# Andreas-Edling/raytracer-rs

Measured on AMD Instinct MI355X. Metric: Mrays/s (whole node) + ms/frame, 1920x1080x64spp thai2.dae, higher is better.
Workload: dtype f32

## Files before the change

### include/mi355rt.h

```cpp
#ifndef MI355RT_H
#define MI355RT_H

#include <stddef.h>
#include <stdint.h>

#ifdef __cplusplus
extern "C" {
#endif

#define MI355RT_OK            0
#define MI355RT_E_INVALID    -1
#define MI355RT_E_NO_DEVICE  -2
#define MI355RT_E_LOAD       -3
#define MI355RT_E_HIP        -4

#define MI355RT_DEFAULT_TRIANGLES_PER_LEAF 70u
#define MI355RT_DEFAULT_STRIPE_ROWS 4u

#define MI355RT_FLAG_FIX_ROW_INDEX  1u
#define MI355RT_FLAG_COUNT_STEPS    2u
#define MI355RT_FLAG_TIME_KERNELS   4u
#define MI355RT_FLAG_OCTREE_SEMANTICS 8u
#define MI355RT_FLAG_TRUE_CLOSEST_HIT 32u
#define MI355RT_FLAG_GROUP_SHARES_DEVICE 16u
#define MI355RT_FLAG_DEVICE_LBVH 64u
#define MI355RT_FLAG_DIRECT_FILM 128u

typedef struct mi355rt_handle mi355rt_handle;

typedef struct mi355rt_material {
    uint32_t kind;
    float rgb[3];
    uint32_t tex_id;
} mi355rt_material;

typedef struct mi355rt_light {
    float pos[3];
    float color[3];
} mi355rt_light;

typedef struct mi355rt_texture {
    uint32_t width, height;
    const float* rgb;
} mi355rt_texture;

typedef struct mi355rt_scene_desc {
    const float* tri_verts;
    const uint32_t* tri_geom;
    uint32_t ntri;
    const mi355rt_material* materials;
    uint32_t nmaterials;
    const mi355rt_light* lights;
    uint32_t nlights;
    const mi355rt_texture* textures;
    uint32_t ntextures;
    float camera_orientation[16];
    float camera_fov_deg;
} mi355rt_scene_desc;

typedef struct mi355rt_config {
    uint32_t width, height;
    uint32_t triangles_per_leaf;
    uint32_t recursions;
    uint32_t spread;
    uint32_t flags;
    uint64_t seed;
    int32_t device;
    uint32_t stripe_rows, stripe_rank, stripe_world;
    uint32_t samples_per_pass;
    uint32_t device_count;
} mi355rt_config;

typedef struct mi355rt_ray_counts {
    uint64_t primary;
    uint64_t bounce;
    uint64_t shadow;
    uint64_t primary_hits;
    uint64_t primary_culled;
    uint64_t nodes_visited;
    uint64_t tris_tested;
    uint64_t trace_launches;
    uint64_t inner_execs;
    uint64_t leaf_execs;
    double trace_ms;
    double total_ms;
    double trace_secondary_ms;
    uint64_t trace_secondary_launches;
    double shader_clock_mhz;
    uint64_t shadow_skipped;
} mi355rt_ray_counts;

void mi355rt_default_config(mi355rt_config* cfg);

int mi355rt_create(const mi355rt_scene_desc* scene, const mi355rt_config* cfg, mi355rt_handle** out);
int mi355rt_create_from_collada_str(const char* doc, size_t len, const char* data_dir,
                                    const mi355rt_config* cfg, mi355rt_handle** out);
int mi355rt_create_from_collada_file(const char* path, const mi355rt_config* cfg, mi355rt_handle** out);
int mi355rt_create_from_scene_file(const char* path, const mi355rt_config* cfg, mi355rt_handle** out);
void mi355rt_destroy(mi355rt_handle* h);

const char* mi355rt_last_error(const mi355rt_handle* h);

uint32_t mi355rt_trace_frame_additive(mi355rt_handle* h);
int mi355rt_render(mi355rt_handle* h, uint32_t spp, mi355rt_ray_counts* counts);
int mi355rt_render_async(mi355rt_handle* h, uint32_t spp);
int mi355rt_last_counts(mi355rt_handle* h, mi355rt_ray_counts* counts);

#define MI355RT_ADAPTIVE_TILE 8u
typedef struct mi355rt_adaptive_config {
    uint32_t min_spp;
    uint32_t max_spp;
    uint32_t batch_spp;
    uint32_t max_rounds;
    float rel_error;
    float abs_floor;
} mi355rt_adaptive_config;

typedef struct mi355rt_adaptive_stats {
    uint32_t rounds;
    uint32_t tiles;
    uint32_t tiles_active_first;
    uint32_t tiles_active_last;
    uint64_t samples_added;
} mi355rt_adaptive_stats;

void mi355rt_adaptive_default_config(mi355rt_adaptive_config* cfg);
int mi355rt_render_adaptive(mi355rt_handle* h, const mi355rt_adaptive_config* cfg, mi355rt_adaptive_stats* stats);
int mi355rt_adaptive_tile_mask(mi355rt_handle* h, const mi355rt_adaptive_config* cfg, uint8_t* out, size_t ntiles);

typedef struct mi355rt_denoise_config {
    uint32_t iterations;
    uint32_t normal_power_log2;
    float sigma_luminance;
    float sigma_depth;
    float sigma_albedo;
} mi355rt_denoise_config;
void mi355rt_denoise_default_config(mi355rt_denoise_config* cfg);
int mi355rt_get_denoised_pixels(mi355rt_handle* h, const mi355rt_denoise_config* cfg, float* rgb, uint32_t* packed, size_t npix);
int mi355rt_film_get_direct(mi355rt_handle* h, float* sum_rgb);
int mi355rt_get_denoised_pixels_split(mi355rt_handle* h, const mi355rt_denoise_config* cfg, float* rgb, uint32_t* packed, size_t npix);
int mi355rt_get_guides(mi355rt_handle* h, float* depth, float* normal3, float* albedo3, uint32_t* prim, size_t npix);

#define MI355RT_DISPLAY_SOURCE_FILM            0u
#define MI355RT_DISPLAY_SOURCE_DENOISED        1u
#define MI355RT_DISPLAY_SOURCE_DENOISED_SPLIT  2u
#define MI355RT_CURVE_REINHARD        0u
#define MI355RT_CURVE_REINHARD_WHITE  1u
#define MI355RT_CURVE_ACES            2u
#define MI355RT_CURVE_CLAMP           3u
#define MI355RT_TRANSFER_REFERENCE    0u
#define MI355RT_TRANSFER_SRGB         1u
#define MI355RT_HIST_BINS 256u

typedef struct mi355rt_luminance_histogram {
    uint32_t bins[MI355RT_HIST_BINS];
    uint32_t empty;
    uint32_t nan;
    uint32_t nonpositive;
    uint32_t max_bits;
} mi355rt_luminance_histogram;

typedef struct mi355rt_display_config {
    uint32_t source, curve, transfer;
    uint32_t auto_exposure;
    float exposure;
    float white;
    float key, low, high;
} mi355rt_display_config;

void mi355rt_display_default_config(mi355rt_display_config* cfg);
int mi355rt_display_histogram(mi355rt_handle* h, uint32_t source, const mi355rt_denoise_config* dn, mi355rt_luminance_histogram* out);
int mi355rt_display_auto_exposure(const mi355rt_luminance_histogram* hist, float key, float low, float high, float* exposure);
int mi355rt_display_srgb_thresholds(float out[255]);
int mi355rt_get_display_pixels(mi355rt_handle* h, const mi355rt_display_config* cfg, const mi355rt_denoise_config* dn,
                               uint32_t* packed, size_t npix, float* exposure_used );

int mi355rt_get_tonemapped_pixels(mi355rt_handle* h, uint32_t* out, size_t n);
int mi355rt_tonemap_owned_rows_device(mi355rt_handle* h, uint32_t* device_out, size_t n);
int mi355rt_tonemap_owned_rows_device_on_stream(mi355rt_handle* h, uint32_t* device_out, size_t n, void* hip_stream);
uint32_t mi355rt_owned_rows(const mi355rt_handle* h);
int mi355rt_owned_row_list(const mi355rt_handle* h, uint32_t* rows, size_t n);

int mi355rt_film_get(mi355rt_handle* h, float* sum_rgb, float* sumsq_rgb, uint32_t* n);
int mi355rt_film_clear(mi355rt_handle* h);
int mi355rt_film_get_pixels(mi355rt_handle* h, float* rgb);
int mi355rt_film_get_estimated_variances(mi355rt_handle* h, float* rgb);

int mi355rt_film_set(mi355rt_handle* h, const float* sum_rgb, const float* sumsq_rgb, const uint32_t* n, const float* direct_rgb, size_t npix);
int mi355rt_film_add(mi355rt_handle* h, const float* sum_rgb, const float* sumsq_rgb, const uint32_t* n, const float* direct_rgb, size_t npix);
int mi355rt_film_save(mi355rt_handle* h, const char* path);
int mi355rt_film_load(mi355rt_handle* h, const char* path, int add);
int mi355rt_film_file_info(const char* path, uint32_t out[8]);

int mi355rt_camera_move_rel(mi355rt_handle* h, float x, float y, float z);
int mi355rt_camera_add_x_angle(mi355rt_handle* h, float radians);
int mi355rt_camera_add_y_angle(mi355rt_handle* h, float radians);
int mi355rt_camera_get(const mi355rt_handle* h, float rot16[16], float orient16[16], float max_xy[2]);
int mi355rt_camera_get_ray(const mi355rt_handle* h, uint32_t u, uint32_t v, float xi1, float xi2, float ray6[6]);

int mi355rt_set_seed(mi355rt_handle* h, uint64_t seed);
int mi355rt_set_flags(mi355rt_handle* h, uint32_t flags);
int mi355rt_set_slices(mi355rt_handle* h, uint32_t slices);
uint32_t mi355rt_get_slices(const mi355rt_handle* h);

int mi355rt_intersect_rays(mi355rt_handle* h, const float* rays6, size_t n, float* tuv, uint32_t* prim);
int mi355rt_occluded_rays(mi355rt_handle* h, const float* rays6, size_t n, uint8_t* blocked);

#define MI355RT_RAYS_HOST   0u
#define MI355RT_RAYS_DEVICE 1u
typedef struct mi355rt_ray_outputs {
    float*    rgb;
    float*    direct;
    float*    tuv;
    uint32_t* prim;
} mi355rt_ray_outputs;
int mi355rt_trace_rays(mi355rt_handle* h, const float* rays6, const uint32_t* keys2 ,
                       size_t n, uint32_t where, const mi355rt_ray_outputs* out);
int mi355rt_render_rays(mi355rt_handle* h, const float* rays6, size_t nrays, uint32_t spp, uint32_t where, mi355rt_ray_counts* counts);

int mi355rt_get_sample_table(const mi355rt_handle* h, float* out);
int mi355rt_debug_sample(mi355rt_handle* h, uint32_t pixel, uint32_t sampleno, float color3[3], float* node_L, size_t nodes);
int mi355rt_debug_numerics(mi355rt_handle* h, const float* a, const float* b, size_t n, float* quot, float* root, float* pow32);
int mi355rt_debug_slab(mi355rt_handle* h, const float* inv_rays6, const float* cubes6, size_t n, uint8_t* hit, float* tmin);
uint32_t mi355rt_tree_nodes(const mi355rt_handle* h);
int mi355rt_debug_speculation(const mi355rt_handle* h, uint64_t out[2]);
int mi355rt_debug_light_map(const float* tri_verts, uint32_t ntri, const float light[3], double pad, uint32_t res, float* out_dist2, double* nearest);

int mi355rt_debug_wide_bvh(const float* tri_verts, uint32_t ntri, uint32_t out[8]);

int mi355rt_accel_stats(const mi355rt_handle* h, uint32_t out[8]);
int mi355rt_bvh_build_info(const mi355rt_handle* h, uint32_t out[2]);
int mi355rt_octree_stats(const mi355rt_handle* h, uint32_t out[8]);
uint32_t mi355rt_device_count(const mi355rt_handle* h);
int mi355rt_debug_gather_rate(mi355rt_handle* h, uint32_t table_nodes, uint32_t steps, double out[3]);
int64_t mi355rt_debug_check_guards(mi355rt_handle* h);
uint64_t mi355rt_hbm_allocated_bytes(const mi355rt_handle* h);
int mi355rt_synchronize(mi355rt_handle* h);

#define MI355RT_COMM_ID_BYTES 128
int mi355rt_comm_unique_id(uint8_t* id128);
int mi355rt_comm_available(mi355rt_handle* h);
int mi355rt_comm_init(mi355rt_handle* h, const uint8_t* id128);
int mi355rt_comm_gather_frame(mi355rt_handle* h, uint32_t root, uint32_t* host_out, size_t n);
int mi355rt_comm_destroy(mi355rt_handle* h);
uint32_t mi355rt_comm_ranks(mi355rt_handle* h);

uint32_t mi355rt_width(const mi355rt_handle* h);
uint32_t mi355rt_height(const mi355rt_handle* h);
uint32_t mi355rt_triangle_count(const mi355rt_handle* h);
uint32_t mi355rt_current_row(const mi355rt_handle* h);

#ifdef __cplusplus
}
#endif
#endif
```

### raytracer-rs_amd/__init__.py

```python
import ctypes as C
import os
import sys
import time
import weakref

import numpy as np

DEFAULT_TRIANGLES_PER_LEAF = 70

FLAG_FIX_ROW_INDEX = 1
FLAG_COUNT_STEPS = 2
FLAG_TIME_KERNELS = 4
FLAG_OCTREE_SEMANTICS = 8
FLAG_GROUP_SHARES_DEVICE = 16
FLAG_TRUE_CLOSEST_HIT = 32
FLAG_DEVICE_LBVH = 64
FLAG_DIRECT_FILM = 128

_HERE = os.path.dirname(os.path.abspath(__file__))
LIB_PATH = os.environ.get("MI355RT_LIB") or os.path.join(_HERE, "libmi355rt.so")
_lib = None


class Material(C.Structure):
    _fields_ = [("kind", C.c_uint32), ("rgb", C.c_float * 3), ("tex_id", C.c_uint32)]


class Light(C.Structure):
    _fields_ = [("pos", C.c_float * 3), ("color", C.c_float * 3)]


class Texture(C.Structure):
    _fields_ = [("width", C.c_uint32), ("height", C.c_uint32), ("rgb", C.POINTER(C.c_float))]


class SceneDesc(C.Structure):
    _fields_ = [
        ("tri_verts", C.POINTER(C.c_float)), ("tri_geom", C.POINTER(C.c_uint32)), ("ntri", C.c_uint32),
        ("materials", C.POINTER(Material)), ("nmaterials", C.c_uint32),
        ("lights", C.POINTER(Light)), ("nlights", C.c_uint32),
        ("textures", C.POINTER(Texture)), ("ntextures", C.c_uint32),
        ("camera_orientation", C.c_float * 16), ("camera_fov_deg", C.c_float),
    ]


class Config(C.Structure):
    _fields_ = [
        ("width", C.c_uint32), ("height", C.c_uint32), ("triangles_per_leaf", C.c_uint32),
        ("recursions", C.c_uint32), ("spread", C.c_uint32), ("flags", C.c_uint32),
        ("seed", C.c_uint64), ("device", C.c_int32),
        ("stripe_rows", C.c_uint32), ("stripe_rank", C.c_uint32), ("stripe_world", C.c_uint32),
        ("samples_per_pass", C.c_uint32), ("device_count", C.c_uint32),
    ]


class RayCounts(C.Structure):
    _fields_ = [
        ("primary", C.c_uint64), ("bounce", C.c_uint64), ("shadow", C.c_uint64), ("primary_hits", C.c_uint64),
        ("primary_culled", C.c_uint64),
        ("nodes_visited", C.c_uint64), ("tris_tested", C.c_uint64), ("trace_launches", C.c_uint64),
        ("inner_execs", C.c_uint64), ("leaf_execs", C.c_uint64),
        ("trace_ms", C.c_double), ("total_ms", C.c_double),
        ("trace_secondary_ms", C.c_double), ("trace_secondary_launches", C.c_uint64), ("shader_clock_mhz", C.c_double),
        ("shadow_skipped", C.c_uint64),
    ]

    def as_dict(self):
        d = {name: getattr(self, name) for name, _ in self._fields_}
        d["total_rays"] = self.primary + self.bounce + self.shadow
        d["traced_rays"] = d["total_rays"] - self.primary_culled - self.shadow_skipped
        return d


ADAPTIVE_TILE = 8


class AdaptiveConfig(C.Structure):
    _fields_ = [("min_spp", C.c_uint32), ("max_spp", C.c_uint32), ("batch_spp", C.c_uint32), ("max_rounds", C.c_uint32),
                ("rel_error", C.c_float), ("abs_floor", C.c_float)]


class AdaptiveStats(C.Structure):
    _fields_ = [("rounds", C.c_uint32), ("tiles", C.c_uint32), ("tiles_active_first", C.c_uint32), ("tiles_active_last", C.c_uint32),
                ("samples_added", C.c_uint64)]

    def as_dict(self):
        return {name: int(getattr(self, name)) for name, _ in self._fields_}


class DenoiseConfig(C.Structure):
    _fields_ = [("iterations", C.c_uint32), ("normal_power_log2", C.c_uint32),
                ("sigma_luminance", C.c_float), ("sigma_depth", C.c_float), ("sigma_albedo", C.c_float)]


HIST_BINS = 256
DISPLAY_SOURCE_FILM, DISPLAY_SOURCE_DENOISED, DISPLAY_SOURCE_DENOISED_SPLIT = 0, 1, 2
CURVE_REINHARD, CURVE_REINHARD_WHITE, CURVE_ACES, CURVE_CLAMP = 0, 1, 2, 3
TRANSFER_REFERENCE, TRANSFER_SRGB = 0, 1


class LuminanceHistogram(C.Structure):
    _fields_ = [("bins", C.c_uint32 * HIST_BINS), ("empty", C.c_uint32), ("nan", C.c_uint32), ("nonpositive", C.c_uint32), ("max_bits", C.c_uint32)]

    def as_dict(self):
        return dict(bins=np.array(self.bins, np.uint32), empty=int(self.empty), nan=int(self.nan), nonpositive=int(self.nonpositive), max_bits=int(self.max_bits))

    @classmethod
    def from_dict(cls, d):
        h = cls()
        bins = np.ascontiguousarray(d["bins"], np.uint32).reshape(HIST_BINS)
        C.memmove(h.bins, bins.ctypes.data, HIST_BINS * 4)
        h.empty, h.nan, h.nonpositive, h.max_bits = (int(d.get(k, 0)) for k in ("empty", "nan", "nonpositive", "max_bits"))
        return h


class DisplayConfig(C.Structure):
    _fields_ = [("source", C.c_uint32), ("curve", C.c_uint32), ("transfer", C.c_uint32), ("auto_exposure", C.c_uint32),
                ("exposure", C.c_float), ("white", C.c_float), ("key", C.c_float), ("low", C.c_float), ("high", C.c_float)]


RAYS_HOST, RAYS_DEVICE = 0, 1


class RayOutputs(C.Structure):
    _fields_ = [("rgb", C.c_void_p), ("direct", C.c_void_p), ("tuv", C.c_void_p), ("prim", C.c_void_p)]


RAY_OUTPUTS = ("rgb", "direct", "tuv", "prim")

_H = C.c_void_p
_F = C.POINTER(C.c_float)
_U = C.POINTER(C.c_uint32)
ABI = [
    ("mi355rt_default_config", None, [C.POINTER(Config)]),
    ("mi355rt_create", C.c_int, [C.POINTER(SceneDesc), C.POINTER(Config), C.POINTER(_H)]),
    ("mi355rt_create_from_collada_str", C.c_int, [C.c_char_p, C.c_size_t, C.c_char_p, C.POINTER(Config), C.POINTER(_H)]),
    ("mi355rt_create_from_collada_file", C.c_int, [C.c_char_p, C.POINTER(Config), C.POINTER(_H)]),
    ("mi355rt_create_from_scene_file", C.c_int, [C.c_char_p, C.POINTER(Config), C.POINTER(_H)]),
    ("mi355rt_destroy", None, [_H]),
    ("mi355rt_last_error", C.c_char_p, [_H]),
    ("mi355rt_trace_frame_additive", C.c_uint32, [_H]),
    ("mi355rt_render", C.c_int, [_H, C.c_uint32, C.POINTER(RayCounts)]),
    ("mi355rt_render_async", C.c_int, [_H, C.c_uint32]),
    ("mi355rt_last_counts", C.c_int, [_H, C.POINTER(RayCounts)]),
    ("mi355rt_adaptive_default_config", None, [C.POINTER(AdaptiveConfig)]),
    ("mi355rt_render_adaptive", C.c_int, [_H, C.POINTER(AdaptiveConfig), C.POINTER(AdaptiveStats)]),
    ("mi355rt_adaptive_tile_mask", C.c_int, [_H, C.POINTER(AdaptiveConfig), C.POINTER(C.c_uint8), C.c_size_t]),
    ("mi355rt_denoise_default_config", None, [C.POINTER(DenoiseConfig)]),
    ("mi355rt_get_denoised_pixels", C.c_int, [_H, C.POINTER(DenoiseConfig), _F, _U, C.c_size_t]),
    ("mi355rt_film_get_direct", C.c_int, [_H, _F]),
    ("mi355rt_get_denoised_pixels_split", C.c_int, [_H, C.POINTER(DenoiseConfig), _F, _U, C.c_size_t]),
    ("mi355rt_get_guides", C.c_int, [_H, _F, _F, _F, _U, C.c_size_t]),
    ("mi355rt_display_default_config", None, [C.POINTER(DisplayConfig)]),
    ("mi355rt_display_histogram", C.c_int, [_H, C.c_uint32, C.POINTER(DenoiseConfig), C.POINTER(LuminanceHistogram)]),
    ("mi355rt_display_auto_exposure", C.c_int, [C.POINTER(LuminanceHistogram), C.c_float, C.c_float, C.c_float, _F]),
    ("mi355rt_display_srgb_thresholds", C.c_int, [_F]),
    ("mi355rt_get_display_pixels", C.c_int, [_H, C.POINTER(DisplayConfig), C.POINTER(DenoiseConfig), _U, C.c_size_t, _F]),
    ("mi355rt_get_tonemapped_pixels", C.c_int, [_H, _U, C.c_size_t]),
    ("mi355rt_tonemap_owned_rows_device", C.c_int, [_H, C.c_void_p, C.c_size_t]),
    ("mi355rt_tonemap_owned_rows_device_on_stream", C.c_int, [_H, C.c_void_p, C.c_size_t, C.c_void_p]),
    ("mi355rt_owned_rows", C.c_uint32, [_H]),
    ("mi355rt_owned_row_list", C.c_int, [_H, _U, C.c_size_t]),
    ("mi355rt_film_get", C.c_int, [_H, _F, _F, _U]),
    ("mi355rt_film_clear", C.c_int, [_H]),
    ("mi355rt_film_set", C.c_int, [_H, _F, _F, _U, _F, C.c_size_t]),
    ("mi355rt_film_add", C.c_int, [_H, _F, _F, _U, _F, C.c_size_t]),
    ("mi355rt_film_save", C.c_int, [_H, C.c_char_p]),
    ("mi355rt_film_load", C.c_int, [_H, C.c_char_p, C.c_int]),
    ("mi355rt_film_file_info", C.c_int, [C.c_char_p, _U]),
    ("mi355rt_film_get_pixels", C.c_int, [_H, _F]),
    ("mi355rt_film_get_estimated_variances", C.c_int, [_H, _F]),
    ("mi355rt_camera_move_rel", C.c_int, [_H, C.c_float, C.c_float, C.c_float]),
    ("mi355rt_camera_add_x_angle", C.c_int, [_H, C.c_float]),
    ("mi355rt_camera_add_y_angle", C.c_int, [_H, C.c_float]),
    ("mi355rt_camera_get", C.c_int, [_H, _F, _F, _F]),
    ("mi355rt_camera_get_ray", C.c_int, [_H, C.c_uint32, C.c_uint32, C.c_float, C.c_float, _F]),
    ("mi355rt_set_seed", C.c_int, [_H, C.c_uint64]),
    ("mi355rt_set_flags", C.c_int, [_H, C.c_uint32]),
    ("mi355rt_set_slices", C.c_int, [_H, C.c_uint32]),
    ("mi355rt_get_slices", C.c_uint32, [_H]),
    ("mi355rt_intersect_rays", C.c_int, [_H, _F, C.c_size_t, _F, _U]),
    ("mi355rt_occluded_rays", C.c_int, [_H, _F, C.c_size_t, C.POINTER(C.c_uint8)]),
    ("mi355rt_trace_rays", C.c_int, [_H, C.c_void_p, C.c_void_p, C.c_size_t, C.c_uint32, C.POINTER(RayOutputs)]),
    ("mi355rt_render_rays", C.c_int, [_H, C.c_void_p, C.c_size_t, C.c_uint32, C.c_uint32, C.POINTER(RayCounts)]),
    ("mi355rt_get_sample_table", C.c_int, [_H, _F]),
    ("mi355rt_debug_sample", C.c_int, [_H, C.c_uint32, C.c_uint32, _F, _F, C.c_size_t]),
    ("mi355rt_debug_numerics", C.c_int, [_H, _F, _F, C.c_size_t, _F, _F, _F]),
    ("mi355rt_debug_slab", C.c_int, [_H, _F, _F, C.c_size_t, C.POINTER(C.c_uint8), _F]),
    ("mi355rt_tree_nodes", C.c_uint32, [_H]),
    ("mi355rt_debug_speculation", C.c_int, [_H, C.POINTER(C.c_uint64)]),
    ("mi355rt_debug_light_map", C.c_int, [_F, C.c_uint32, _F, C.c_double, C.c_uint32, _F, C.POINTER(C.c_double)]),
    ("mi355rt_debug_wide_bvh", C.c_int, [_F, C.c_uint32, _U]),
    ("mi355rt_accel_stats", C.c_int, [_H, _U]),
    ("mi355rt_octree_stats", C.c_int, [_H, _U]),
    ("mi355rt_bvh_build_info", C.c_int, [_H, _U]),
    ("mi355rt_device_count", C.c_uint32, [_H]),
    ("mi355rt_synchronize", C.c_int, [_H]),
    ("mi355rt_comm_unique_id", C.c_int, [C.POINTER(C.c_uint8)]),
    ("mi355rt_comm_available", C.c_int, [_H]),
    ("mi355rt_comm_init", C.c_int, [_H, C.POINTER(C.c_uint8)]),
    ("mi355rt_comm_gather_frame", C.c_int, [_H, C.c_uint32, _U, C.c_size_t]),
    ("mi355rt_comm_destroy", C.c_int, [_H]),
    ("mi355rt_comm_ranks", C.c_uint32, [_H]),
    ("mi355rt_hbm_allocated_bytes", C.c_uint64, [_H]),
    ("mi355rt_debug_check_guards", C.c_int64, [_H]),
    ("mi355rt_debug_gather_rate", C.c_int, [_H, C.c_uint32, C.c_uint32, C.POINTER(C.c_double)]),
    ("mi355rt_width", C.c_uint32, [_H]),
    ("mi355rt_height", C.c_uint32, [_H]),
    ("mi355rt_triangle_count", C.c_uint32, [_H]),
    ("mi355rt_current_row", C.c_uint32, [_H]),
]


def lib():
    global _lib
    if _lib is None:
        if not os.path.exists(LIB_PATH):
            raise ImportError(
                "libmi355rt.so is not built (%s); run __graft_entry__.build() — there is no CPU fallback" % LIB_PATH)
        if "torch" in sys.modules:
            try:
                sys.modules["torch"].cuda.is_available()
            except Exception:
                pass
        L = C.CDLL(LIB_PATH)
        for name, res, args in ABI:
            fn = getattr(L, name)
            fn.restype = res
            fn.argtypes = args
        _lib = L
    return _lib


def _fp(a):
    return a.ctypes.data_as(_F)


def _up(a):
    return a.ctypes.data_as(_U)


def _is_tensor(a):
    t = sys.modules.get("torch")
    return t is not None and isinstance(a, t.Tensor)


def _ray_array(a, name, cols, dtype, rows=None):
    want = np.dtype(dtype).name
    if _is_tensor(a):
        if a.device.type != "cuda":
            raise ValueError("%s: a torch tensor must live on the handle's GPU (it is on %s); pass a numpy array for host memory" % (name, a.device))
        if str(a.dtype).replace("torch.", "") not in ((want, "int32") if want == "uint32" else (want,)):
            raise TypeError("%s: dtype must be %s, not %s" % (name, want, a.dtype))
        shape, contiguous, addr, dev = tuple(a.shape), a.is_contiguous(), a.data_ptr(), True
    elif isinstance(a, np.ndarray):
        if a.dtype != np.dtype(dtype):
            raise TypeError("%s: dtype must be %s, not %s" % (name, want, a.dtype))
        shape, contiguous, addr, dev = a.shape, a.flags["C_CONTIGUOUS"], a.ctypes.data, False
    else:
        raise TypeError("%s: a numpy array or a torch tensor, not %s" % (name, type(a).__name__))
    if len(shape) != 2 or shape[1] != cols or (rows is not None and shape[0] != rows):
        raise ValueError("%s: shape must be (%s, %d), not %s" % (name, "n" if rows is None else rows, cols, tuple(shape)))
    if not contiguous:
        raise ValueError("%s: must be C-contiguous" % name)
    return addr, shape[0], dev


def default_config(width=1024, height=768, **kw):
    cfg = Config()
    lib().mi355rt_default_config(C.byref(cfg))
    cfg.width, cfg.height = int(width), int(height)
    for k, v in kw.items():
        if not hasattr(cfg, k):
            raise TypeError("unknown config field %r" % k)
# ... 287 lines not shown
        else:
            self._check(lib().mi355rt_tonemap_owned_rows_device(self._h, C.c_void_p(device_ptr), n))

    def intersect_rays(self, rays6):
        rays6 = np.ascontiguousarray(rays6, np.float32).reshape(-1, 6)
        n = rays6.shape[0]
        tuv = np.zeros((n, 3), np.float32); prim = np.zeros(n, np.uint32)
        self._check(lib().mi355rt_intersect_rays(self._h, _fp(rays6), n, _fp(tuv), _up(prim)))
        return tuv, prim

    def trace_rays(self, rays6, keys=None, want=("rgb",)):
        want = tuple(want)
        if not want or any(w not in RAY_OUTPUTS for w in want) or len(set(want)) != len(want):
            raise ValueError("want: a non-empty selection of %s without repeats, not %r" % (RAY_OUTPUTS, want))
        addr, n, dev = _ray_array(rays6, "rays6", 6, np.float32)
        kaddr = None
        if keys is not None:
            kaddr, _, kdev = _ray_array(keys, "keys", 2, np.uint32, rows=n)
            if kdev != dev:
                raise ValueError("keys must live where rays6 lives (both numpy arrays, or both tensors on the GPU)")
        res, o = {}, RayOutputs()
        if dev:
            import torch
            torch.cuda.current_stream(rays6.device).synchronize()
            for w in want:
                res[w] = torch.zeros((n,) if w == "prim" else (n, 3), dtype=torch.int32 if w == "prim" else torch.float32, device=rays6.device)
                setattr(o, w, res[w].data_ptr())
            torch.cuda.current_stream(rays6.device).synchronize()
        else:
            for w in want:
                res[w] = np.zeros(n, np.uint32) if w == "prim" else np.zeros((n, 3), np.float32)
                setattr(o, w, res[w].ctypes.data)
        self._check(lib().mi355rt_trace_rays(self._h, addr, kaddr, n, RAYS_DEVICE if dev else RAYS_HOST, C.byref(o)))
        return res

    def render_rays(self, rays6, spp):
        spp = int(spp)
        if spp < 1:
            raise ValueError("spp must be >= 1")
        addr, n, dev = _ray_array(rays6, "rays6", 6, np.float32, rows=self.width * self.height * spp)
        if dev:
            import torch
            torch.cuda.current_stream(rays6.device).synchronize()
        rc = RayCounts()
        self._check(lib().mi355rt_render_rays(self._h, addr, n, spp, RAYS_DEVICE if dev else RAYS_HOST, C.byref(rc)))
        return rc

    def occluded_rays(self, rays6):
        rays6 = np.ascontiguousarray(rays6, np.float32).reshape(-1, 6)
        n = rays6.shape[0]
        out = np.zeros(n, np.uint8)
        self._check(lib().mi355rt_occluded_rays(self._h, _fp(rays6), n, out.ctypes.data_as(C.POINTER(C.c_uint8))))
        return out

    def sample_table(self):
        out = np.zeros((65536, 3), np.float32)
        self._check(lib().mi355rt_get_sample_table(self._h, _fp(out)))
        return out

    def debug_sample(self, pixel, sampleno):
        nodes = lib().mi355rt_tree_nodes(self._h)
        color = np.zeros(3, np.float32); node_l = np.zeros((nodes, 3), np.float32)
        self._check(lib().mi355rt_debug_sample(self._h, pixel, sampleno, _fp(color), _fp(node_l), nodes))
        return color, node_l

    def debug_numerics(self, a, b):
        a = np.ascontiguousarray(a, np.float32); b = np.ascontiguousarray(b, np.float32)
        q = np.zeros_like(a); r = np.zeros_like(a); p = np.zeros_like(a)
        self._check(lib().mi355rt_debug_numerics(self._h, _fp(a), _fp(b), a.size, _fp(q), _fp(r), _fp(p)))
        return q, r, p

    def debug_slab(self, inv_rays6, cubes6):
        r = np.ascontiguousarray(inv_rays6, np.float32).reshape(-1, 6); c = np.ascontiguousarray(cubes6, np.float32).reshape(-1, 6)
        assert r.shape == c.shape
        hit = np.zeros(r.shape[0], np.uint8); tmin = np.zeros(r.shape[0], np.float32)
        self._check(lib().mi355rt_debug_slab(self._h, _fp(r), _fp(c), r.shape[0], hit.ctypes.data_as(C.POINTER(C.c_uint8)), _fp(tmin)))
        return hit.astype(bool), tmin

    def accel_stats(self):
        out = np.zeros(8, np.uint32)
        self._check(lib().mi355rt_accel_stats(self._h, _up(out)))
        return dict(nodes=int(out[0]), leaves=int(out[1]), max_depth=int(out[2]), max_leaf=int(out[3]),
                    node_bytes=int(out[4]), tri_bytes=int(out[5]), bvh_build_ms=int(out[6]) / 1000.0, octree_build_ms=int(out[7]) / 1000.0)

    def bvh_build_info(self):
        out = np.zeros(2, np.uint32)
        self._check(lib().mi355rt_bvh_build_info(self._h, _up(out)))
        return dict(on_device=bool(out[0]), device_ms=int(out[1]) / 1000.0)

    def octree_stats(self):
        out = np.zeros(8, np.uint32)
        self._check(lib().mi355rt_octree_stats(self._h, _up(out)))
        return dict(nodes=int(out[0]), inner=int(out[1]), leaves=int(out[2]), empty=int(out[3]), depth=int(out[4]), tri_refs=int(out[5]))

    @property
    def triangle_count(self):
        return lib().mi355rt_triangle_count(self._h)

    @property
    def current_row(self):
        return lib().mi355rt_current_row(self._h)


def _finish(code, handle, keep=None):
    if code != 0:
        raise RuntimeError((lib().mi355rt_last_error(None) or b"").decode() or "mi355rt error %d" % code)
    return RayTracer(handle.value, keep)


def create_raytracer(collada_doc, triangles_per_leaf, width, height, data_dir=None, **cfg_kw):
    cfg = default_config(width, height, triangles_per_leaf=triangles_per_leaf, **cfg_kw)
    doc = collada_doc.encode() if isinstance(collada_doc, str) else bytes(collada_doc)
    h = C.c_void_p()
    code = lib().mi355rt_create_from_collada_str(doc, len(doc), data_dir.encode() if data_dir else None, C.byref(cfg), C.byref(h))
    return _finish(code, h)


def create_raytracer_from_file(collada_filename, triangles_per_leaf, width, height, **cfg_kw):
    cfg = default_config(width, height, triangles_per_leaf=triangles_per_leaf, **cfg_kw)
    h = C.c_void_p()
    code = lib().mi355rt_create_from_collada_file(str(collada_filename).encode(), C.byref(cfg), C.byref(h))
    return _finish(code, h)


def create_raytracer_from_scene_file(scene_filename, triangles_per_leaf, width, height, **cfg_kw):
    cfg = default_config(width, height, triangles_per_leaf=triangles_per_leaf, **cfg_kw)
    h = C.c_void_p()
    code = lib().mi355rt_create_from_scene_file(str(scene_filename).encode(), C.byref(cfg), C.byref(h))
    return _finish(code, h)


def create_raytracer_from_arrays(scene, triangles_per_leaf, width, height, **cfg_kw):
    cfg = default_config(width, height, triangles_per_leaf=triangles_per_leaf, **cfg_kw)
    verts = np.ascontiguousarray(scene["tri_verts"], np.float32).reshape(-1)
    geom = np.ascontiguousarray(scene["tri_geom"], np.uint32)
    nm = len(scene["mat_kind"])
    mats = (Material * max(nm, 1))()
    for i in range(nm):
        mats[i].kind = int(scene["mat_kind"][i]); mats[i].tex_id = int(scene["mat_tex"][i])
        for c in range(3):
            mats[i].rgb[c] = float(scene["mat_rgb"][i][c])
    nl = len(scene["lights"])
    lights = (Light * max(nl, 1))()
    for i in range(nl):
        for c in range(3):
            lights[i].pos[c] = float(scene["lights"][i][c]); lights[i].color[c] = float(scene["lights"][i][3 + c])
    nt = len(scene["textures"])
    texs = (Texture * max(nt, 1))()
    keep = [verts, geom, mats, lights, texs]
    for i, t in enumerate(scene["textures"]):
        arr = np.ascontiguousarray(t, np.float32)
        keep.append(arr)
        texs[i].height, texs[i].width = arr.shape[0], arr.shape[1]
        texs[i].rgb = _fp(arr)
    sd = SceneDesc()
    sd.tri_verts = _fp(verts); sd.tri_geom = _up(geom); sd.ntri = geom.size
    sd.materials = mats; sd.nmaterials = nm; sd.lights = lights; sd.nlights = nl
    sd.textures = texs; sd.ntextures = nt
    for i in range(16):
        sd.camera_orientation[i] = float(scene["camera_matrix"][i])
    sd.camera_fov_deg = float(scene["camera_fov"])
    h = C.c_void_p()
    code = lib().mi355rt_create(C.byref(sd), C.byref(cfg), C.byref(h))
    return _finish(code, h, keep)


def film_file_info(path):
    out = (C.c_uint32 * 8)()
    if lib().mi355rt_film_file_info(os.fsencode(path), out) != 0:
        raise RuntimeError((lib().mi355rt_last_error(None) or b"").decode() or "mi355rt_film_file_info failed")
    return dict(version=int(out[0]), width=int(out[1]), height=int(out[2]), planes=int(out[3]), seed=int(out[4]) | int(out[5]) << 32, flags=int(out[6]))


def debug_light_map(tri_verts, light, pad, res):
    v = np.ascontiguousarray(tri_verts, np.float32).reshape(-1, 9)
    l = np.ascontiguousarray(light, np.float32).reshape(3)
    out = np.zeros((6, res, res), np.float32); nearest = C.c_double(0.0)
    code = lib().mi355rt_debug_light_map(_fp(v), v.shape[0], _fp(l), float(pad), int(res), _fp(out), C.byref(nearest))
    if code != 0:
        raise RuntimeError("mi355rt_debug_light_map failed: %d" % code)
    return out, nearest.value


def debug_wide_bvh(tri_verts):
    v = np.ascontiguousarray(tri_verts, np.float32).reshape(-1, 9)
    out = (C.c_uint32 * 8)()
    code = lib().mi355rt_debug_wide_bvh(_fp(v), v.shape[0], out)
    if code != 0:
        raise RuntimeError("mi355rt_debug_wide_bvh failed: %d" % code)
    keys = ("wide_nodes", "binary_nodes", "stack_need", "binary_depth", "children", "tris_once_wide", "bad_boxes", "tris_once_binary")
    return dict(zip(keys, (int(x) for x in out)))


def comm_unique_id():
    buf = (C.c_uint8 * 128)()
    if lib().mi355rt_comm_unique_id(buf) != 0:
        raise RuntimeError((lib().mi355rt_last_error(None) or b"").decode() or "mi355rt_comm_unique_id failed")
    return bytes(buf)


class Stats:

    def __init__(self):
        self.last_iteration = time.perf_counter()
        self.fps_sum = 0.0
        self.primrays_per_sec_sum = 0.0
        self.num_measurements = 0

    def stats(self, num_primary_rays):
        now = time.perf_counter()
        dt = now - self.last_iteration
        self.last_iteration = now
        fps = 1.0 / dt
        self.fps_sum += fps
        prs = num_primary_rays / dt
        self.primrays_per_sec_sum += prs
        self.num_measurements += 1
        return "fps: %s  primary rays/s: %d" % (fps, int(prs))

    def mean_stats(self):
        return "mean fps: %s  mean primary rays/s: %s" % (
            self.fps_sum / self.num_measurements, self.primrays_per_sec_sum / self.num_measurements)


class stats:
    Stats = Stats
```

### raytracer-rs_amd/csrc/capi.cpp

```cpp
#include <cmath>
#include <cstdio>
#include <cstring>
#include <memory>
#include <string>
#include <vector>
#include "display.hpp"
#include "lightmap.hpp"
#include "../../include/mi355rt.h"
#include "group.hpp"
#include "renderer.hpp"

using namespace mi355rt;

namespace mi355rt { bool comm_unique_id(uint8_t* id128, std::string& err); }

struct mi355rt_handle {
    std::unique_ptr<DeviceGroup> g;
    Renderer* r;
    std::string error;
};

namespace {
thread_local std::string g_create_error;

int finish_create(const SceneData& scene, const mi355rt_config* cfg, mi355rt_handle** out)
{
    int code = MI355RT_E_INVALID;
    std::string err;
    std::unique_ptr<DeviceGroup> g = DeviceGroup::create(scene, *cfg, err, code);
    if (!g) { g_create_error = err; return code; }
    Renderer* r = g->primary();
    *out = new mi355rt_handle{ std::move(g), r, std::string() };
    return MI355RT_OK;
}
int bad(const char* msg) { g_create_error = msg; return MI355RT_E_INVALID; }

bool adaptive_args_ok(mi355rt_handle* h, const mi355rt_adaptive_config* c)
{
    if (!h) return false;
    const char* e = nullptr;
    if (h->g->size() > 1) e = "adaptive sampling: not available on a device group (config.device_count > 1)";
    else if (!c) e = "adaptive sampling: null config";
    else if (c->min_spp < 2) e = "adaptive sampling: min_spp must be >= 2";
    else if (c->max_spp < c->min_spp) e = "adaptive sampling: max_spp must be >= min_spp";
    else if (c->batch_spp < 1) e = "adaptive sampling: batch_spp must be >= 1";
    else if (!std::isfinite(c->rel_error) || c->rel_error < 0.0f) e = "adaptive sampling: rel_error must be finite and >= 0";
    else if (!std::isfinite(c->abs_floor) || c->abs_floor < 0.0f) e = "adaptive sampling: abs_floor must be finite and >= 0";
    if (!e) return true;
    h->r->last_error = e;
    return false;
}

bool denoise_handle_ok(mi355rt_handle* h, size_t npix)
{
    if (!h) return false;
    const char* e = nullptr;
    if (h->g->size() > 1) e = "denoise: not available on a device group (config.device_count > 1)";
    else if (h->r->cfg.stripe_world > 1) e = "denoise: not available on a striped handle (stripe_world > 1): a stripe's neighbours belong to other ranks";
    else if (npix < (size_t)h->r->cfg.width * h->r->cfg.height) e = "denoise: output buffer too small: npix must be >= width * height";
    if (!e) return true;
    h->r->last_error = e;
    return false;
}
bool denoise_config_ok(mi355rt_handle* h, const mi355rt_denoise_config* c)
{
    const char* e = nullptr;
    auto sigma_ok = [](float s) { return std::isfinite(s) && s > 0.0f; };
    if (!c) e = "denoise: null config";
    else if (c->iterations > 10) e = "denoise: iterations must be <= 10";
    else if (c->normal_power_log2 > 10) e = "denoise: normal_power_log2 must be <= 10";
    else if (!sigma_ok(c->sigma_luminance)) e = "denoise: sigma_luminance must be finite and > 0";
    else if (!sigma_ok(c->sigma_depth)) e = "denoise: sigma_depth must be finite and > 0";
    else if (!sigma_ok(c->sigma_albedo)) e = "denoise: sigma_albedo must be finite and > 0";
    if (!e) return true;
    h->r->last_error = e;
    return false;
}
bool display_handle_ok(mi355rt_handle* h, uint32_t source)
{
    if (!h) return false;
    const char* e = nullptr;
    if (h->g->size() > 1) e = "display: not available on a device group (config.device_count > 1)";
    else if (h->r->cfg.stripe_world > 1) e = "display: not available on a striped handle (stripe_world > 1): add the stripes into one handle first";
    else if (source > MI355RT_DISPLAY_SOURCE_DENOISED_SPLIT) e = "display: unknown source";
    else if (source == MI355RT_DISPLAY_SOURCE_DENOISED_SPLIT && !h->r->has_direct_film()) e = "display: source DENOISED_SPLIT needs a handle created with MI355RT_FLAG_DIRECT_FILM";
    if (!e) return true;
    h->r->last_error = e;
    return false;
}
const char* display_key_range_error(float key, float low, float high)
// ... 478 lines not shown
    return h->g->set_seed(seed) ? MI355RT_OK : MI355RT_E_HIP;
}
int mi355rt_set_flags(mi355rt_handle* h, uint32_t flags)
{
    if (!h) return MI355RT_E_INVALID;
    return h->g->set_flags(flags) ? MI355RT_OK : MI355RT_E_INVALID;
}

int mi355rt_set_slices(mi355rt_handle* h, uint32_t slices)
{
    if (!h || slices < 1 || slices > 8) return MI355RT_E_INVALID;
    h->g->set_slices(slices);
    return MI355RT_OK;
}
uint32_t mi355rt_get_slices(const mi355rt_handle* h) { return h ? h->r->slices : 0; }

int mi355rt_intersect_rays(mi355rt_handle* h, const float* rays6, size_t n, float* tuv, uint32_t* prim)
{
    if (!h || (n && (!rays6 || !tuv || !prim))) return MI355RT_E_INVALID;
    return h->r->intersect(rays6, n, tuv, prim, nullptr) ? MI355RT_OK : MI355RT_E_HIP;
}
int mi355rt_occluded_rays(mi355rt_handle* h, const float* rays6, size_t n, uint8_t* blocked)
{
    if (!h || (n && (!rays6 || !blocked))) return MI355RT_E_INVALID;
    return h->r->intersect(rays6, n, nullptr, nullptr, blocked) ? MI355RT_OK : MI355RT_E_HIP;
}

int mi355rt_trace_rays(mi355rt_handle* h, const float* rays6, const uint32_t* keys2, size_t n, uint32_t where, const mi355rt_ray_outputs* out)
{
    if (!ray_call_ok(h, "mi355rt_trace_rays", rays6, n, where)) return MI355RT_E_INVALID;
    if (!out || (!out->rgb && !out->direct && !out->tuv && !out->prim)) { h->r->last_error = "mi355rt_trace_rays: out is NULL or every output pointer in it is NULL"; return MI355RT_E_INVALID; }
    if (n > 0xFFFFFFFFull) { h->r->last_error = "mi355rt_trace_rays: n must fit 32 bits"; return MI355RT_E_INVALID; }
    return h->r->trace_rays(rays6, keys2, n, where == MI355RT_RAYS_DEVICE, *out) ? MI355RT_OK : MI355RT_E_HIP;
}

int mi355rt_render_rays(mi355rt_handle* h, const float* rays6, size_t nrays, uint32_t spp, uint32_t where, mi355rt_ray_counts* counts)
{
    if (!ray_call_ok(h, "mi355rt_render_rays", rays6, nrays, where)) return MI355RT_E_INVALID;
    const char* e = nullptr;
    if (spp == 0) e = "mi355rt_render_rays: spp must be >= 1";
    else if (nrays != (size_t)h->r->cfg.width * h->r->cfg.height * spp) e = "mi355rt_render_rays: nrays must equal width * height * spp";
    if (e) { h->r->last_error = e; return MI355RT_E_INVALID; }
    const bool ok = h->r->render_rays(rays6, spp, where == MI355RT_RAYS_DEVICE);
    if (counts) *counts = h->r->counts;
    return ok ? MI355RT_OK : MI355RT_E_HIP;
}

int mi355rt_get_sample_table(const mi355rt_handle* h, float* out)
{
    if (!h || !out) return MI355RT_E_INVALID;
    std::memcpy(out, h->r->table.data(), h->r->table.size() * sizeof(float));
    return MI355RT_OK;
}

int mi355rt_debug_sample(mi355rt_handle* h, uint32_t pixel, uint32_t sampleno, float color3[3], float* node_L, size_t nodes)
{
    if (!h || !color3 || !node_L) return MI355RT_E_INVALID;
    return h->r->debug_sample(pixel, sampleno, color3, node_L, nodes) ? MI355RT_OK : MI355RT_E_HIP;
}
int mi355rt_debug_numerics(mi355rt_handle* h, const float* a, const float* b, size_t n, float* quot, float* root, float* pow32)
{
    if (!h || (n && (!a || !b || !quot || !root || !pow32))) return MI355RT_E_INVALID;
    return h->r->debug_numerics(a, b, n, quot, root, pow32) ? MI355RT_OK : MI355RT_E_HIP;
}
int mi355rt_debug_slab(mi355rt_handle* h, const float* inv_rays6, const float* cubes6, size_t n, uint8_t* hit, float* tmin)
{
    if (!h || (n && (!inv_rays6 || !cubes6 || !hit || !tmin))) return MI355RT_E_INVALID;
    return h->r->debug_slab(inv_rays6, cubes6, n, hit, tmin) ? MI355RT_OK : MI355RT_E_HIP;
}
uint32_t mi355rt_tree_nodes(const mi355rt_handle* h) { return h ? h->r->nodes_per_sample : 0u; }
int mi355rt_debug_speculation(const mi355rt_handle* h, uint64_t out[2])
{
    if (!h || !out) return MI355RT_E_INVALID;
    h->r->speculation_stats(out);
    return MI355RT_OK;
}
int mi355rt_debug_light_map(const float* tri_verts, uint32_t ntri, const float light[3], double pad, uint32_t res, float* out_dist2, double* nearest)
{
    if ((ntri && !tri_verts) || !light || !out_dist2 || res == 0 || res > 4096 || !(pad >= 0.0)) return MI355RT_E_INVALID;
    mi355rt::LightMap lm;
    mi355rt::build_light_map(tri_verts, ntri, light, pad, res, lm);
    std::memcpy(out_dist2, lm.dist2.data(), lm.dist2.size() * sizeof(float));
    if (nearest) *nearest = lm.nearest;
    return MI355RT_OK;
}

namespace {
struct WideWalk {
    const mi355rt::Bvh& b; std::vector<uint32_t> seen; uint32_t children = 0, bad_boxes = 0;
    void below(int32_t ref, double mn[3], double mx[3])
    {
        for (int a = 0; a < 3; ++a) { mn[a] = 1e300; mx[a] = -1e300; }
        if (ref < 0) {
            const uint32_t code = ~(uint32_t)ref, first = code >> 3, cnt = (code & 7u) + 1u;
            for (uint32_t t = first; t < first + cnt && t < b.tris.size(); ++t) {
                const mi355rt::BvhTri& r = b.tris[t];
                if (r.prim < seen.size()) ++seen[r.prim];
                for (int v = 0; v < 3; ++v) for (int a = 0; a < 3; ++a) {
                    const double x = (double)r.v0[a] + (v == 1 ? (double)r.e1[a] : v == 2 ? (double)r.e2[a] : 0.0);
                    mn[a] = std::min(mn[a], x); mx[a] = std::max(mx[a], x);
                }
            }
            return;
        }
        const mi355rt::BvhNode4& o = b.nodes4[(size_t)ref];
        const uint32_t cbm = (o.bases & 0xFFFFFu) - 128u, nb = ~(((o.bases >> 20) | ((o.ew >> 24) << 12)) << 3);
        const uint32_t lo[3] = { o.lox, o.loy, o.loz }, hi[3] = { o.hix, o.hiy, o.hiz };
        for (int i = 0; i < 4; ++i) {
            if (((lo[0] >> (8 * i)) & 0xFFu) > ((hi[0] >> (8 * i)) & 0xFFu)) continue;
            ++children;
            const uint32_t t = (o.meta >> (8 * i)) & 0xFFu;
            const int32_t cref = (t & 0x80u) ? (int32_t)(cbm + t) : (int32_t)(nb - t);
            double cmn[3], cmx[3];
            below(cref, cmn, cmx);
            for (int a = 0; a < 3; ++a) {
                const double scale = std::ldexp(1.0, (int)((o.ew >> (8 * a)) & 0xFFu) - 127);
                const double blo = (double)o.org[a] + (double)((lo[a] >> (8 * i)) & 0xFFu) * scale, bhi = (double)o.org[a] + (double)((hi[a] >> (8 * i)) & 0xFFu) * scale;
                if (cmn[a] <= cmx[a] && (blo > cmn[a] || bhi < cmx[a])) { ++bad_boxes; break; }
                mn[a] = std::min(mn[a], cmn[a]); mx[a] = std::max(mx[a], cmx[a]);
            }
        }
    }
};
}

int mi355rt_debug_wide_bvh(const float* tri_verts, uint32_t ntri, uint32_t out[8])
{
    if ((ntri && !tri_verts) || !out) return MI355RT_E_INVALID;
    std::vector<uint32_t> geom(std::max(ntri, 1u), 0u);
    mi355rt::Bvh b;
    mi355rt::build_bvh(tri_verts, geom.data(), ntri, b);
    mi355rt::build_wide(b);
    for (int k = 0; k < 8; ++k) out[k] = 0u;
    out[1] = (uint32_t)b.nodes.size(); out[3] = b.max_depth;
    if (b.nodes4.empty()) return MI355RT_OK;
    out[0] = (uint32_t)b.nodes4.size(); out[2] = b.stack_need4;
    WideWalk w{ b, std::vector<uint32_t>(ntri, 0u) };
    double mn[3], mx[3];
    w.below(0, mn, mx);
    out[4] = w.children; out[6] = w.bad_boxes;
    for (uint32_t c : w.seen) out[5] += c == 1u ? 1u : 0u;
    std::vector<uint32_t> seen2(ntri, 0u);
    std::vector<int32_t> st(1, b.root);
    while (!st.empty()) {
        const int32_t r = st.back(); st.pop_back();
        if (r < 0) { const uint32_t code = ~(uint32_t)r, first = code >> 3, cnt = (code & 7u) + 1u; for (uint32_t t = first; t < first + cnt && t < b.tris.size(); ++t) if (b.tris[t].prim < ntri) ++seen2[b.tris[t].prim]; }
        else { st.push_back(b.nodes[(size_t)r].child0); st.push_back(b.nodes[(size_t)r].child1); }
    }
    for (uint32_t c : seen2) out[7] += c == 1u ? 1u : 0u;
    return MI355RT_OK;
}

int mi355rt_accel_stats(const mi355rt_handle* h, uint32_t out[8])
{
    if (!h || !out) return MI355RT_E_INVALID;
    const Bvh& b = h->r->bvh;
    out[0] = (uint32_t)b.nodes.size(); out[1] = b.leaves; out[2] = b.max_depth; out[3] = b.max_leaf;
    out[4] = (uint32_t)(b.nodes.size() * sizeof(BvhNode)); out[5] = (uint32_t)(b.tris.size() * sizeof(BvhTri));
    out[6] = (uint32_t)(h->r->build_ms_[0] * 1000.0); out[7] = (uint32_t)(h->r->build_ms_[1] * 1000.0);
    return MI355RT_OK;
}
int mi355rt_bvh_build_info(const mi355rt_handle* h, uint32_t out[2])
{
    if (!h || !out) return MI355RT_E_INVALID;
    out[0] = h->r->bvh_on_device_ ? 1u : 0u; out[1] = (uint32_t)(h->r->lbvh_device_ms_ * 1000.0);
    return MI355RT_OK;
}
int mi355rt_octree_stats(const mi355rt_handle* h, uint32_t out[8])
{
    if (!h || !out) return MI355RT_E_INVALID;
    std::memcpy(out, h->r->oct_stats_, sizeof h->r->oct_stats_);
    return MI355RT_OK;
}
uint32_t mi355rt_device_count(const mi355rt_handle* h) { return h ? (uint32_t)h->g->size() : 0u; }

int mi355rt_debug_gather_rate(mi355rt_handle* h, uint32_t table_nodes, uint32_t steps, double out[3])
{
    if (!h || !out) return MI355RT_E_INVALID;
    return h->r->debug_gather_rate(table_nodes, steps, out) ? MI355RT_OK : MI355RT_E_HIP;
}

int64_t mi355rt_debug_check_guards(mi355rt_handle* h)
{
    if (!h) return -1;
    int64_t bad = 0;
    for (size_t i = 0; i < h->g->size(); ++i) { const long b = h->g->device(i)->check_guards(); if (b < 0) return -1; bad += b; }
    return bad;
}

uint64_t mi355rt_hbm_allocated_bytes(const mi355rt_handle* h)
{
    if (!h) return 0;
    uint64_t b = 0;
    for (size_t i = 0; i < h->g->size(); ++i) b += h->g->device(i)->hbm_allocated_bytes();
    return b;
}

int mi355rt_synchronize(mi355rt_handle* h)
{
    if (!h) return MI355RT_E_INVALID;
    return h->g->synchronize() ? MI355RT_OK : MI355RT_E_HIP;
}

int mi355rt_comm_unique_id(uint8_t* id128)
{
    if (!id128) return bad("null argument");
    std::string err;
    if (!comm_unique_id(id128, err)) { g_create_error = err; return MI355RT_E_HIP; }
    return MI355RT_OK;
}
int mi355rt_comm_available(mi355rt_handle* h)
{
    if (!h) return MI355RT_E_INVALID;
    if (h->g->size() > 1) { h->r->last_error = "a device group gathers inside the process; RCCL communicators are for one-device handles"; return MI355RT_E_INVALID; }
    return h->r->comm_available() ? MI355RT_OK : MI355RT_E_HIP;
}
int mi355rt_comm_init(mi355rt_handle* h, const uint8_t* id128)
{
    if (!h || !id128) return MI355RT_E_INVALID;
    if (h->g->size() > 1) { h->r->last_error = "a device group gathers inside the process; RCCL communicators are for one-device handles"; return MI355RT_E_INVALID; }
    return h->r->comm_init(id128) ? MI355RT_OK : MI355RT_E_HIP;
}
int mi355rt_comm_gather_frame(mi355rt_handle* h, uint32_t root, uint32_t* host_out, size_t n)
{
    if (!h) return MI355RT_E_INVALID;
    return h->r->comm_gather(root, host_out, n) ? MI355RT_OK : MI355RT_E_HIP;
}
int mi355rt_comm_destroy(mi355rt_handle* h)
{
    if (!h) return MI355RT_E_INVALID;
    h->r->comm_destroy();
    return MI355RT_OK;
}
uint32_t mi355rt_comm_ranks(mi355rt_handle* h) { return h ? h->r->comm_ranks() : 0u; }

uint32_t mi355rt_width(const mi355rt_handle* h) { return h ? h->r->cfg.width : 0u; }
uint32_t mi355rt_height(const mi355rt_handle* h) { return h ? h->r->cfg.height : 0u; }
uint32_t mi355rt_triangle_count(const mi355rt_handle* h) { return h ? h->r->ntri : 0u; }
uint32_t mi355rt_current_row(const mi355rt_handle* h) { return h ? h->r->current_row : 0u; }

}
```

### raytracer-rs_amd/csrc/device_types.hpp

```cpp
#pragma once
#include <cstdint>
#include <hip/hip_vector_types.h>

namespace mi355rt {

constexpr uint32_t kNumSamples = 65536;
constexpr uint32_t kSampleMax = 65535;
constexpr uint32_t kMaxRecursions = 3;
constexpr uint32_t kMaxLevels = kMaxRecursions + 1;

constexpr uint32_t kRayRecordBytes = 32;
constexpr uint32_t kShards = 64;
constexpr uint32_t kMaxRounds = kMaxRecursions + 2;
constexpr uint32_t kCullRects = 16;
constexpr uint32_t kMaxCursors = 64;
constexpr uint32_t kCtrlWordsPerRound = kMaxCursors * 16384;
constexpr uint32_t kShadeCursorOffset = 128;
constexpr uint32_t kConfirmCursorOffset = 64;
constexpr uint32_t kLiveCountOffset = 192;

struct DMaterial { float r, g, b; uint32_t kind_tex; };
struct DLight { float px, py, pz, cr, cg, cb;
                float tail2;
                float pad; };
struct DTexture { uint32_t width, height; uint64_t offset; };

struct DScene {
    const void* nodes;
    const void* tris;
    const void* normals;
    const DMaterial* materials;
    const DLight* lights;
    const DTexture* textures;
    const float* texels;
    const void* table;
    const void* oct_nodes;
    const uint32_t* oct_leaf_tris;
    const void* prim_tris;
    const int2* oct_info;
    const uint32_t* tri_home;
    const float* light_maps;
    uint32_t light_map_res;
    int32_t root;
    uint32_t nlights;
    uint32_t ntri;
    uint32_t oct_single_leaf;
    float oct_root[6];
};

struct DCamera {
    float rot[16];
    float origin[3];
    float max_x, max_y;
    uint32_t width, height;
    uint32_t cull_valid;
    float cull_rect[kCullRects][4];
    const uint32_t* cull_mask;
    float mask_x0, mask_y0, mask_inv_cx, mask_inv_cy;
    const uint2* tile_ofs;
    const uint2* tile_entries;
    uint32_t tile_cols, tile_rg, tile_nblocks;
};
constexpr uint32_t kCullGrid = 1024;

struct DPass {
    const uint32_t* rows;
    size_t qstride;
    uint2* slot_ps;
    uint32_t* hit_prim;
    uint32_t row0;
    uint32_t row_wrap;
    uint32_t npix;
    uint32_t row_group, row_group_shift;
    uint32_t nsamples;
    uint32_t spp;
    uint32_t sample_group;
    uint32_t seed;
    uint32_t flags;
    uint32_t recursions, spread;
    uint32_t nodes_per_sample;
    uint32_t nslots;
    uint32_t level_first[kMaxLevels + 1];
    uint32_t use_explicit, explicit_pixel, explicit_sampleno;
    uint32_t chunk;
    uint32_t nchunks;
    uint32_t region;
    uint32_t stack_depth;
    uint32_t list_cap;
    uint32_t tail_chunks;
    const uint32_t* block_culled;
    uint32_t cull_blocks;
    uint32_t* live;
    uint32_t* live_count;
    uint32_t live_cap;
    const uint8_t* tile_active;
    uint32_t tiles_x;
    const float* ray_in;
    const uint32_t* ray_keys;
    float4* ray_hit;
    uint32_t ray_mode, ray_base, ray_npix;
};
constexpr uint32_t kAdaptiveTile = 8;
struct AdaptiveArgs {
    uint32_t width, height, tiles_x, tiles_y;
    uint32_t stripe_rows, stripe_world, stripe_rank;
    uint32_t min_spp, max_spp, batch_spp;
    float rel_error, abs_floor;
};
constexpr uint32_t kDnHit = 1u, kDnEmpty = 2u, kDnUnknown = 4u;
struct DenoiseArgs {
    uint32_t width, height;
    uint32_t step;
    uint32_t normal_power_log2;
    float sigma_luminance, sigma_depth, sigma_albedo;
};
constexpr uint32_t kDisplayHistWords = 260u, kDisplayHistBlock = 1024u;
struct DisplayArgs {
    uint32_t curve, transfer;
    float exposure;
    float white2;
};

struct DCounters {
    unsigned long long bounce, shadow, primary_hits, nodes_visited, tris_tested;
    unsigned long long inner_execs, leaf_execs;
    unsigned int overflow;
    unsigned int pad;
    unsigned long long primary_culled;
    unsigned long long shadow_skipped;
    unsigned long long t_first_end, t_last_end, t_sum_end, t_start, n_waves;
    unsigned long long lanes_inner, lanes_leaf, lanes_done, lane_samples;
    unsigned long long t_sum_cycles, t_sum_real;
    unsigned long long visits_below[6];
    unsigned long long refills, refill_passes, refill_rays;
};

}
```

### raytracer-rs_amd/csrc/group.cpp

```cpp
#include "group.hpp"
#include <algorithm>
#include <cstring>
#include <thread>

namespace mi355rt {

std::unique_ptr<DeviceGroup> DeviceGroup::create(const SceneData& scene, const mi355rt_config& cfg_in, std::string& err, int& code)
{
    std::unique_ptr<DeviceGroup> g(new DeviceGroup());
    mi355rt_config cfg = cfg_in;
    const uint32_t n = cfg.device_count <= 1 ? 1u : cfg.device_count;
    code = MI355RT_E_INVALID;
    if (n > 64) { err = "device_count > 64"; return nullptr; }
    if (n > 1 && cfg.stripe_world > 1) { err = "a device group deals the rows itself: stripe_world must be <= 1 when device_count > 1"; return nullptr; }
    for (uint32_t i = 0; i < n; ++i) {
        mi355rt_config c = cfg;
        c.device_count = 1;
        if (n > 1) {
            c.device = (cfg.flags & MI355RT_FLAG_GROUP_SHARES_DEVICE) ? cfg.device : cfg.device + (int32_t)i;
            if (c.stripe_rows == 0) c.stripe_rows = MI355RT_DEFAULT_STRIPE_ROWS;
            c.stripe_rank = i; c.stripe_world = n;
        }
        std::unique_ptr<Renderer> r = Renderer::create(scene, c, err, code);
        if (!r) { if (n > 1) err = "device " + std::to_string(c.device) + ": " + err; return nullptr; }
        g->devs_.push_back(std::move(r));
    }
    if (n > 1) {
        for (uint32_t i = 1; i < n; ++i) {
            const int a = g->devs_[0]->cfg.device, b = g->devs_[i]->cfg.device;
            if (a == b) continue;
            int can = 0;
            if (hipDeviceCanAccessPeer(&can, b, a) == hipSuccess && can && hipSetDevice(b) == hipSuccess) {
                hipError_t e = hipDeviceEnablePeerAccess(a, 0);
                if (e != hipSuccess && e != hipErrorPeerAccessAlreadyEnabled) (void)hipGetLastError();
            }
        }
        for (uint32_t i = 0; i < n; ++i)
            if (!g->devs_[i]->gather_prepare(i == 0)) { err = g->devs_[i]->last_error; code = MI355RT_E_HIP; return nullptr; }
    }
    code = MI355RT_OK;
    return g;
}

uint32_t DeviceGroup::trace_frame_additive()
{
    error_.clear();
    uint32_t ret = 0;
    for (size_t i = 0; i < devs_.size(); ++i) {
        ret = devs_[i]->trace_frame_additive();
        if (ret == 0) { fail_from(i); return 0; }
    }
    counts_from_render_ = false;
    return ret;
}

bool DeviceGroup::render(uint32_t spp, bool wait)
{
    error_.clear();
    if (devs_.size() == 1) { counts_from_render_ = false; return primary()->render(spp, wait); }
    std::vector<char> ok(devs_.size(), 0);
    std::vector<std::thread> th;
    for (size_t i = 0; i < devs_.size(); ++i) th.emplace_back([&, i] { ok[i] = devs_[i]->render(spp) ? 1 : 0; });
    for (auto& t : th) t.join();
    counts_ = mi355rt_ray_counts{};
    for (size_t i = 0; i < devs_.size(); ++i) {
        if (!ok[i]) return fail_from(i);
        const mi355rt_ray_counts& c = devs_[i]->counts;
        counts_.primary += c.primary; counts_.bounce += c.bounce; counts_.shadow += c.shadow; counts_.shadow_skipped += c.shadow_skipped; counts_.primary_hits += c.primary_hits;
        counts_.primary_culled += c.primary_culled; counts_.nodes_visited += c.nodes_visited; counts_.tris_tested += c.tris_tested;
        counts_.trace_launches += c.trace_launches; counts_.inner_execs += c.inner_execs; counts_.leaf_execs += c.leaf_execs;
        counts_.trace_ms += c.trace_ms; counts_.total_ms = std::max(counts_.total_ms, c.total_ms);
        counts_.trace_secondary_ms += c.trace_secondary_ms; counts_.trace_secondary_launches += c.trace_secondary_launches; counts_.shader_clock_mhz = std::max(counts_.shader_clock_mhz, c.shader_clock_mhz);
    }
    counts_from_render_ = true;
    return true;
}

bool DeviceGroup::last_counts(mi355rt_ray_counts& out)
{
    error_.clear();
    if (devs_.size() == 1) return primary()->last_counts(out);
    if (counts_from_render_) { out = counts_; return true; }
    out = mi355rt_ray_counts{};
    for (size_t i = 0; i < devs_.size(); ++i) {
        mi355rt_ray_counts c{};
        if (!devs_[i]->last_counts(c)) return fail_from(i);
        out.primary += c.primary; out.bounce += c.bounce; out.shadow += c.shadow; out.shadow_skipped += c.shadow_skipped; out.primary_hits += c.primary_hits;
        out.primary_culled += c.primary_culled; out.nodes_visited += c.nodes_visited; out.tris_tested += c.tris_tested;
        out.trace_launches += c.trace_launches; out.inner_execs += c.inner_execs; out.leaf_execs += c.leaf_execs;
        out.trace_ms += c.trace_ms; out.total_ms = std::max(out.total_ms, c.total_ms);
        out.trace_secondary_ms += c.trace_secondary_ms; out.trace_secondary_launches += c.trace_secondary_launches; out.shader_clock_mhz = std::max(out.shader_clock_mhz, c.shader_clock_mhz);
    }
    return true;
}

bool DeviceGroup::get_tonemapped(uint32_t* out, size_t n)
{
    error_.clear();
    if (devs_.size() == 1) return primary()->get_tonemapped(out, n);
    Renderer* root = primary();
    for (size_t i = 1; i < devs_.size(); ++i) {
        Renderer* d = devs_[i].get();
        if (!d->tonemap_to_gather_slot()) return fail_from(i);
        const size_t bytes = d->owned_rows.size() * (size_t)d->cfg.width * 4;
        hipError_t e = bytes ? hipMemcpyPeerAsync(root->gather_slot((uint32_t)i), root->cfg.device, d->gather_slot((uint32_t)i), d->cfg.device, bytes, d->stream()) : hipSuccess;
        if (e == hipSuccess) e = hipEventRecord(d->gather_event(), d->stream());
        if (e != hipSuccess) { error_ = std::string("stripe copy to device 0: ") + hipGetErrorString(e); return false; }
    }
    if (!root->tonemap_to_gather_slot()) return fail_from(0);
    for (size_t i = 1; i < devs_.size(); ++i) {
        hipError_t e = hipStreamWaitEvent(root->stream(), devs_[i]->gather_event(), 0);
        if (e != hipSuccess) { error_ = std::string("hipStreamWaitEvent: ") + hipGetErrorString(e); return false; }
    }
    if (!root->finish_gather(out, n)) return fail_from(0);
    return true;
}

bool DeviceGroup::film_get(float* sum, float* sumsq, uint32_t* n)
{
    error_.clear();
    if (devs_.size() == 1) return primary()->film_get(sum, sumsq, n);
    const uint32_t w = primary()->cfg.width; const size_t npix = (size_t)w * primary()->cfg.height;
    std::vector<float> ts(sum ? npix * 3 : 0), tq(sumsq ? npix * 3 : 0); std::vector<uint32_t> tn(n ? npix : 0);
    for (size_t i = 0; i < devs_.size(); ++i) {
        if (!devs_[i]->film_get(sum ? ts.data() : nullptr, sumsq ? tq.data() : nullptr, n ? tn.data() : nullptr)) return fail_from(i);
        for (uint32_t r : devs_[i]->owned_rows) {
            if (sum) std::memcpy(sum + (size_t)r * w * 3, ts.data() + (size_t)r * w * 3, (size_t)w * 12);
            if (sumsq) std::memcpy(sumsq + (size_t)r * w * 3, tq.data() + (size_t)r * w * 3, (size_t)w * 12);
            if (n) std::memcpy(n + (size_t)r * w, tn.data() + (size_t)r * w, (size_t)w * 4);
        }
    }
    return true;
}

bool DeviceGroup::film_get_direct(float* sum)
{
    error_.clear();
    if (devs_.size() == 1) return primary()->film_get_direct(sum);
    const uint32_t w = primary()->cfg.width; const size_t npix = (size_t)w * primary()->cfg.height;
    std::vector<float> t(npix * 3);
    for (size_t i = 0; i < devs_.size(); ++i) {
        if (!devs_[i]->film_get_direct(t.data())) return fail_from(i);
        for (uint32_t r : devs_[i]->owned_rows) std::memcpy(sum + (size_t)r * w * 3, t.data() + (size_t)r * w * 3, (size_t)w * 12);
    }
    return true;
}

bool DeviceGroup::film_stat(bool variances, float* rgb)
{
    error_.clear();
    if (devs_.size() == 1) return primary()->film_stat(variances, rgb);
    const uint32_t w = primary()->cfg.width; const size_t npix = (size_t)w * primary()->cfg.height;
    std::vector<float> t(npix * 3);
    for (size_t i = 0; i < devs_.size(); ++i) {
        if (!devs_[i]->film_stat(variances, t.data())) return fail_from(i);
        for (uint32_t r : devs_[i]->owned_rows) std::memcpy(rgb + (size_t)r * w * 3, t.data() + (size_t)r * w * 3, (size_t)w * 12);
    }
    return true;
}

bool DeviceGroup::film_clear()
{
    error_.clear();
    for (size_t i = 0; i < devs_.size(); ++i) if (!devs_[i]->film_clear()) return fail_from(i);
    return true;
}
bool DeviceGroup::film_put(const Renderer::FilmPlanes& in, bool add)
{
    error_.clear();
    for (size_t i = 0; i < devs_.size(); ++i) if (!devs_[i]->film_put(in, add)) return fail_from(i);
// ... 27 lines not shown
```

### raytracer-rs_amd/csrc/kernels.hip

```cpp
#include <hip/hip_runtime.h>
#include <algorithm>
#include <stdint.h>
#include <stdlib.h>
#include <map>
#include <mutex>
#include <utility>
#include "device_math.hpp"
#include "device_types.hpp"
#include "kernels.hpp"
#include "traverse.hpp"

namespace mi355rt {

typedef const uint32_t __attribute__((address_space(4))) * const_u1_ptr;
constexpr int kBlock = 256;
constexpr int kWavesPerBlock = kBlock / 64;
constexpr uint32_t kMiss = 0xFFFFFFFFu;
constexpr int kPrimaryBlocks = 7;
#ifndef MI355RT_WIDE_BLOCKS
#define MI355RT_WIDE_BLOCKS 5
#endif
constexpr int kConfirmBlocks = 5;
constexpr int kShadePBlocks = 5;
constexpr int kShadePWBlocks = 4;
constexpr int kShadeSWBlocks = 5;
constexpr int kShadeSBlocks = 7;
constexpr int kInnerStepsPerIteration = 2;
constexpr uint32_t kLeafThreshold = 16;
constexpr uint32_t kRefillThreshold = 24;
constexpr uint32_t kRefillPrimary = 48;

__device__ __forceinline__ uint32_t global_wave_id() { return blockIdx.x * kWavesPerBlock + (threadIdx.x >> 6); }

constexpr uint32_t kCursorStride = kCtrlWordsPerRound / kMaxCursors;
constexpr uint32_t kMaxTries = 8u;
static_assert(kCursorStride == 16384 && kShadeCursorOffset == 2 * kConfirmCursorOffset && kLiveCountOffset == 3 * kConfirmCursorOffset, "cursor layout (device_types.hpp) and the reset loop of resolve_kernel");
struct PullState { bool first = true; uint32_t shard = 0u, tries = 0u, part = 0xFFFFFFFFu; };
struct LiveLists { const uint32_t* list = nullptr; const uint32_t* count = nullptr; uint32_t cap = 0u; };
__device__ __forceinline__ LiveLists live_lists(const DPass& ps) { LiveLists l; l.list = ps.live; l.count = ps.live_count; l.cap = ps.live_cap; return l; }
constexpr uint32_t kWholeChunk = 0xFFFFFFFFu;

constexpr uint32_t kTailSplitShift = 2;
__device__ __forceinline__ bool pull_chunk(uint32_t* cursor, uint32_t nchunks, PullState& st, uint32_t& chunk, uint32_t tail = 0u, const LiveLists live = LiveLists())
{
    if (live.list != nullptr) {
        if (st.first) { st.first = false; st.shard = global_wave_id() % kMaxCursors; }
        while (st.tries < kMaxTries) {
            const uint32_t len = ((const_u1_ptr)(uintptr_t)live.count)[(size_t)st.shard * kCursorStride + kLiveCountOffset];
            uint32_t v = 0xFFFFFFFFu;
            if (len != 0u) { if (lane_id() == 0) v = atomicAdd(&cursor[(size_t)st.shard * kCursorStride], 1u); v = bcast_first(v); }
            uint32_t j = v; st.part = kWholeChunk;
            if (tail != 0u && v != 0xFFFFFFFFu) {
                const uint32_t head = len - (tail < len ? tail : len);
                if (v >= head) { const uint32_t jj = v - head; j = head + (jj >> kTailSplitShift); st.part = jj & ((1u << kTailSplitShift) - 1u); }
            }
            if (j < len) { chunk = ((const_u1_ptr)(uintptr_t)live.list)[(size_t)st.shard * live.cap + j]; return true; }
            st.shard = (st.shard + 1u) % kMaxCursors;
            ++st.tries;
        }
        return false;
    }
    if (st.first) { st.first = false; st.shard = global_wave_id() % kMaxCursors; }
    while (st.tries < kMaxTries) {
        uint32_t v = 0u;
        if (lane_id() == 0) v = atomicAdd(&cursor[(size_t)st.shard * kCursorStride], 1u);
        v = bcast_first(v);
        if (tail != 0u) {
            const uint32_t len = st.shard < nchunks ? (nchunks - st.shard + kMaxCursors - 1u) / kMaxCursors : 0u;
            const uint32_t head = len - (tail < len ? tail : len);
            uint32_t j = v; st.part = kWholeChunk;
            if (v >= head) { const uint32_t jj = v - head; j = head + (jj >> kTailSplitShift); st.part = jj & ((1u << kTailSplitShift) - 1u); }
            if (j < len) { chunk = st.shard + j * kMaxCursors; return true; }
        } else {
            const uint32_t c = st.shard + v * kMaxCursors;
            if (c < nchunks) { chunk = c; return true; }
        }
        st.shard = (st.shard + 1u) % kMaxCursors;
        ++st.tries;
    }
    return false;
}

constexpr uint32_t kNT = 4;
typedef float v4f_t __attribute__((ext_vector_type(4)));
template <uint32_t BIT> __device__ __forceinline__ float4 ld4(const float4* p)
{
    if constexpr ((kNT >> BIT) & 1u) { const v4f_t v = __builtin_nontemporal_load((const v4f_t*)p); return make_float4(v.x, v.y, v.z, v.w); }
    else return *p;
}
template <uint32_t BIT> __device__ __forceinline__ void st4(float4* p, float4 a)
{
    if constexpr ((kNT >> BIT) & 1u) { v4f_t v; v.x = a.x; v.y = a.y; v.z = a.z; v.w = a.w; __builtin_nontemporal_store(v, (v4f_t*)p); }
// ... 505 lines not shown

template <bool PRIMARY>
__global__ __launch_bounds__(kBlock, kConfirmBlocks) void confirm_kernel(DScene sc, DCamera cam, DPass ps, const float4* __restrict__ in_q, const uint2* __restrict__ in_counts,
                                                         float4* __restrict__ hits, uint32_t* cursor, float* __restrict__ slot_L, const uint32_t* __restrict__ film_n, uint32_t shadow_only)
{
    __shared__ uint32_t s_list[kWavesPerBlock][2][128];
    const int lane = lane_id();
    uint32_t* list_r = s_list[threadIdx.x >> 6][0];
    uint32_t* list_s = s_list[threadIdx.x >> 6][1];
    uint32_t cnt = 0u;
    PullState pull; uint32_t chunk = 0u;
    while (pull_chunk(cursor, ps.nchunks, pull, chunk, 0u, PRIMARY ? LiveLists() : live_lists(ps))) {
        uint32_t n_rad = 0u, n_sh = 0u;
        if (PRIMARY) {
            n_rad = min(ps.chunk, ps.nsamples - chunk * ps.chunk);
            if (chunk_culled(cam, ps, chunk, n_rad)) continue;
        } else { const uint2 n = in_counts[chunk]; n_rad = n.x; n_sh = n.y; }
        const uint32_t n_tot = n_rad + n_sh;
        for (uint32_t it = shadow_only ? n_rad : 0u; it < n_tot; it += 64u) {
            const uint32_t i = it + (uint32_t)lane;
            const bool valid = i < n_tot;
            const uint32_t r = valid ? (uint32_t)record_index(ps, chunk, i, n_rad) : 0u;
            const bool hit = valid && ld1<3>(&ps.hit_prim[r]) != kMiss;
                uint32_t n_new;
            const uint32_t pos = wave_append(hit, cnt, n_new);
            if (hit) { list_r[pos] = r | (i >= n_rad ? 0x80000000u : 0u); if (PRIMARY) list_s[pos] = chunk * ps.chunk + i; }
            __builtin_amdgcn_wave_barrier();
            if (cnt >= 64u) {
                cnt -= 64u;
                const uint32_t code = list_r[cnt + (uint32_t)lane];
                const uint32_t si = PRIMARY ? list_s[cnt + (uint32_t)lane] : 0u;
                __builtin_amdgcn_wave_barrier();
                confirm_record<PRIMARY>(sc, cam, ps, code & 0x7FFFFFFFu, si, (code >> 31) != 0u, in_q, hits, slot_L, film_n);
            }
        }
    }
    if ((uint32_t)lane < cnt) {
        const uint32_t code = list_r[lane];
        confirm_record<PRIMARY>(sc, cam, ps, code & 0x7FFFFFFFu, PRIMARY ? list_s[lane] : 0u, (code >> 31) != 0u, in_q, hits, slot_L, film_n);
    }
}

__device__ __forceinline__ void hemisphere_walk(const float4* __restrict__ table, const f3 n, uint32_t& jx, float4& tv)
{
    for (uint32_t guard = 0u; tv.x * n.x + tv.y * n.y + tv.z * n.z <= 0.0f && guard < kNumSamples; guard += 4u) {
        const uint32_t j1 = jx + 1u == kSampleMax ? 0u : jx + 1u;
        const uint32_t j2 = j1 + 1u == kSampleMax ? 0u : j1 + 1u;
        const uint32_t j3 = j2 + 1u == kSampleMax ? 0u : j2 + 1u;
        const uint32_t j4 = j3 + 1u == kSampleMax ? 0u : j3 + 1u;
        const float4 t1 = table[j1], t2 = table[j2], t3 = table[j3], t4 = table[j4];
        const bool r1 = t1.x * n.x + t1.y * n.y + t1.z * n.z <= 0.0f, r2 = t2.x * n.x + t2.y * n.y + t2.z * n.z <= 0.0f;
        const bool r3 = t3.x * n.x + t3.y * n.y + t3.z * n.z <= 0.0f;
        const uint32_t left = kNumSamples - guard;
        if (!r1 || left == 1u) { tv = t1; jx = j1; break; }
        if (!r2 || left == 2u) { tv = t2; jx = j2; break; }
        if (!r3 || left == 3u) { tv = t3; jx = j3; break; }
        tv = t4; jx = j4;
    }
}

constexpr uint32_t kSortBins = 8;
__device__ __forceinline__ uint32_t dir_bin(const f3 d) { return (d.x < 0.0f ? 1u : 0u) | (d.y < 0.0f ? 2u : 0u) | (d.z < 0.0f ? 4u : 0u); }

__device__ __forceinline__ bool light_proves_unoccluded(const DScene& sc, uint32_t li, const DLight& lt, const f3 l)
{
    const uint32_t R = sc.light_map_res;
    if (R == 0u) return false;
    const float l2 = l.x * l.x + l.y * l.y + l.z * l.z;
    const float vx = -l.x, vy = -l.y, vz = -l.z;
    const float ax = fabsf(vx), ay = fabsf(vy), az = fabsf(vz);
    uint32_t m; float vm, va, vb;
    if (ax >= ay && ax >= az) { m = 0u; vm = vx; va = vy; vb = vz; }
    else if (ay >= az) { m = 1u; vm = vy; va = vx; vb = vz; }
    else { m = 2u; vm = vz; va = vx; vb = vy; }
    const float am = fabsf(vm);
    if (!(am > 0.0f) || !(l2 < 3.0e38f)) return false;
    const float fR = (float)R, u = div_rn(va, am), v = div_rn(vb, am);
    const int i = min(max((int)((u * 0.5f + 0.5f) * fR), 0), (int)R - 1), j = min(max((int)((v * 0.5f + 0.5f) * fR), 0), (int)R - 1);
    const uint32_t face = 2u * m + (vm < 0.0f ? 1u : 0u);
    const float bound = sc.light_maps[((size_t)(li * 6u + face) * R + (uint32_t)i) * R + (uint32_t)j];
    return (l2 * 0.98011f < bound) & (l2 * 1.0002e-4f < lt.tail2);
}

template <bool PRIMARY, class List, bool WALK = false, bool RASTER = false, bool RAYS = false>
__device__ __forceinline__ void shade_chunk(const DScene& sc, const DCamera& cam, const DPass& ps, uint32_t level, uint32_t chunk, const List list,
                                            const float4* __restrict__ in_q, uint32_t in_nrad, uint32_t& out_nrad, uint32_t& out_nshadow,
                                            const float4* __restrict__ hits,
                                            float4* __restrict__ out_q, uint2* __restrict__ out_counts,
                                            float* __restrict__ slot_L, uint32_t* __restrict__ sample_slot,
                                            const uint32_t* __restrict__ film_n, DCounters* counters,
                                            unsigned long long& acc_bounce, unsigned long long& acc_shadow, unsigned long long& acc_hits,
                                            float4* lds_hits = nullptr, unsigned long long* acc_tris = nullptr)
{
    const int lane = lane_id();
    {
        uint32_t n_rad = PRIMARY ? min(ps.chunk, ps.nsamples - chunk * ps.chunk) : in_nrad;
        const size_t base = (size_t)chunk * ps.region;
        if (PRIMARY && !RAYS && chunk_culled(cam, ps, chunk, n_rad)) {
            if (ps.block_culled == nullptr) for (uint32_t i = (uint32_t)lane; i < n_rad; i += 64u) sample_slot[chunk * ps.chunk + i] = kMiss;
            acc_hits += (unsigned long long)chunk_active_samples(cam, ps, chunk, n_rad) << 32;
            n_rad = 0u;
        }
        uint32_t cnt = 0u;
        for (uint32_t it = 0; it < n_rad; it += 64u) {
            const uint32_t i = it + (uint32_t)lane;
            bool valid;
            float4 found = make_float4(0, 0, 0, 0);
            if (RASTER) {
                f3 ro, rd; float bt, bu, bv; uint32_t bprim;
                bool in = i < n_rad;
                if (ps.tile_active != nullptr && in) { uint32_t s, p; sample_of(ps, chunk * ps.chunk + i, s, p); in = pixel_active(ps, cam.width, pass_pixel(ps, cam.width, p)); }
                const uint32_t tested = raster_tile(sc, cam, ps, film_n, chunk, it, in, ro, rd, bt, bu, bv, bprim);
                if (acc_tris) *acc_tris += (unsigned long long)tested * (unsigned long long)__popcll(__ballot(in));
                valid = in && bprim != kMiss;
                found = make_float4(bt, bu, bv, __uint_as_float(bprim));
            } else valid = i < n_rad && ld1<2>(&ps.hit_prim[base + i]) != kMiss;
            uint32_t n_new;
            const uint32_t pos = wave_append(valid, cnt, n_new);
            if (valid) list[pos] = i;
            if (RASTER && valid) lds_hits[pos] = found;
            if (PRIMARY && i < n_rad) st1<2>(&sample_slot[chunk * ps.chunk + i], valid ? chunk * ps.chunk + pos : kMiss);
            if constexpr (RAYS) { if (ps.ray_hit != nullptr && i < n_rad && !valid) ps.ray_hit[chunk * ps.chunk + i] = make_float4(0.0f, 0.0f, 0.0f, __uint_as_float(kMiss)); }
        }
        if (PRIMARY) {
            const uint32_t planes = ps.nodes_per_sample * sc.nlights, total = cnt * 3u;
            for (uint32_t q = sc.nlights; q < planes; ++q) {
                float* z = slot_L + 3ull * ((size_t)q * ps.nslots + (size_t)chunk * ps.chunk);
                float4* z4 = (float4*)z;
                for (uint32_t k = (uint32_t)lane; k < total / 4u; k += 64u) st4<2>(&z4[k], make_float4(0.0f, 0.0f, 0.0f, 0.0f));
                for (uint32_t k = (total & ~3u) + (uint32_t)lane; k < total; k += 64u) z[k] = 0.0f;
            }
        }
        __builtin_amdgcn_wave_barrier();
        uint32_t out_front = 0u, out_back = 0u, dropped = 0u, skipped = 0u;
        for (uint32_t j = 0; j < cnt; j += 64u) {
            bool active = j + (uint32_t)lane < cnt;
            const bool in_batch = active;
            f3 o = mk3(0, 0, 0), d = mk3(0, 0, 1), hp = mk3(0, 0, 0), n = mk3(0, 0, 1);
            uint32_t slot = 0u, node = 0u, pixel = 0u, sampleno = 0u, geom = 0u;
            float4 h = make_float4(0, 0, 0, 0);
            if (active) {
                const uint32_t i = list[j + (uint32_t)lane];
                h = RASTER ? lds_hits[j + (uint32_t)lane] : ld4<2>(&hits[base + i]);
                if (PRIMARY) {
                    slot = chunk * ps.chunk + j + (uint32_t)lane;
                    primary_sample<RAYS>(cam, ps, film_n, chunk * ps.chunk + i, pixel, sampleno, o, d);
                } else {
                    const float4 r0 = ld4<2>(&in_q[base + i]), r1 = ld4<2>(&in_q[ps.qstride + base + i]);
                    o = mk3(r0.x, r0.y, r0.z); d = mk3(r0.w, r1.x, r1.y);
                    slot = __float_as_uint(r1.z); node = (__float_as_uint(r1.w) >> 8) & 0xFFFFu;
                    const uint2 px = ps.slot_ps[slot];
                    pixel = px.x; sampleno = px.y;
                }
                if (PRIMARY && level < ps.recursions) ps.slot_ps[slot] = make_uint2(pixel, sampleno);
                if (WALK) {
                    float wt = h.x, wu = h.y, wv = h.z; uint32_t wprim = __float_as_uint(h.w);
                    confirm_walk(sc, o, d, wt, wu, wv, wprim);
                    h = make_float4(wt, wu, wv, __uint_as_float(wprim));
                    active = wprim != kMiss;
                }
                if constexpr (RAYS) { if (ps.ray_hit != nullptr) ps.ray_hit[chunk * ps.chunk + i] = active ? h : make_float4(0.0f, 0.0f, 0.0f, __uint_as_float(kMiss)); }
            }
            if (WALK) dropped += (uint32_t)__popcll(__ballot(j + (uint32_t)lane < cnt && !active));
            if (active) {
                hp = add3(o, sscale(h.x, d));
                const float4 nn = ((const float4*)sc.normals)[__float_as_uint(h.w)];
                n = mk3(nn.x, nn.y, nn.z);
                geom = __float_as_uint(nn.w);
            }
            for (uint32_t li = 0; li < sc.nlights; ++li) {
                bool want = false, is_free = false;
                f3 c = mk3(0, 0, 0);
                if (active) {
                    const DLight lt = sc.lights[li];
                    const f3 l = sub3(mk3(lt.px, lt.py, lt.pz), hp);
                    const f3 ln = normalized3(l);
                    const float ndl = dot3(n, ln);
                    if (!(ndl < 0.0f)) {
                        want = true;
                        is_free = light_proves_unoccluded(sc, li, lt, l);
                        const DMaterial m = sc.materials[geom];
                        f3 diffuse = mk3(m.r, m.g, m.b);
                        if (m.kind_tex & 0x80000000u) diffuse = fetch_texel(sc, m.kind_tex & 0x7FFFFFFFu, h.y, h.z);
                        const f3 view = normalized3(d);
                        const f3 refl = sub3(sscale(2.0f * ndl, n), ln);
                        const float spec = pow32(dot3(view, refl));
                        c = mk3((diffuse.x * ndl + spec) * lt.cr, (diffuse.y * ndl + spec) * lt.cg, (diffuse.z * ndl + spec) * lt.cb);
                    }
                }
                uint32_t n_new;
                const bool ray = want && !is_free;
                skipped += (uint32_t)__popcll(__ballot(want && is_free));
                const uint32_t oi = wave_append(ray, out_back, n_new);
                if (want && (!ray || out_front + oi < ps.region)) {
                    const uint32_t term = 3u * ((node * sc.nlights + li) * ps.nslots + slot);
                    if (ray) st4<2>(&out_q[base + (ps.region - 1u - oi)], make_float4(hp.x, hp.y, hp.z, __uint_as_float(term)));
                    float* dst = slot_L + term;
                    dst[0] = c.x; dst[1] = c.y; dst[2] = c.z;
                } else if (PRIMARY && in_batch) {
                    float* dst = slot_L + 3ull * ((size_t)li * ps.nslots + (size_t)chunk * ps.chunk + j + (uint32_t)lane);
                    dst[0] = 0.0f; dst[1] = 0.0f; dst[2] = 0.0f;
                }
            }
            if (level < ps.recursions) {
                const uint32_t k = ps.spread * (ps.recursions - level);
                const uint32_t index_in_level = node - ps.level_first[level];
                for (uint32_t ci = 0; ci < k; ci += 2u) {
                    const bool two = ci + 1u < k;
                    const uint32_t child0 = ps.level_first[level + 1] + index_in_level * k + ci, child1 = child0 + 1u;
                    f3 bo0 = mk3(0, 0, 0), bd0 = mk3(0, 0, 1), bo1 = bo0, bd1 = bd0;
                    if (active) {
                        const float4* __restrict__ table = (const float4*)sc.table;
                        uint32_t a0 = pixel, a1 = sampleno, a2 = 1u + child0, a3 = ps.seed;
                        pcg4d(a0, a1, a2, a3);
                        uint32_t jx0 = __umulhi(a0, 65535u), jx1 = jx0;
                        if (two) {
                            uint32_t b0 = pixel, b1 = sampleno, b2 = 1u + child1, b3 = ps.seed;
                            pcg4d(b0, b1, b2, b3);
                            jx1 = __umulhi(b0, 65535u);
                        }
                        float4 tv0 = table[jx0], tv1 = table[jx1];
                        hemisphere_walk(table, n, jx0, tv0);
                        if (two) hemisphere_walk(table, n, jx1, tv1);
                        bd0 = mk3(tv0.x, tv0.y, tv0.z); bo0 = add3(hp, sscale(0.00001f, bd0));
                        bd1 = mk3(tv1.x, tv1.y, tv1.z); bo1 = add3(hp, sscale(0.00001f, bd1));
                    }
                    uint32_t pos[2] = { 0u, 0u };
                    const uint32_t key0 = active ? dir_bin(bd0) : kSortBins, key1 = (active && two) ? dir_bin(bd1) : kSortBins;
                    for (uint32_t b = 0; b < kSortBins; ++b) {
                        const unsigned long long m0 = __ballot(key0 == b), m1 = __ballot(key1 == b);
                        if (key0 == b) pos[0] = out_front + (uint32_t)__popcll(m0 & lanemask_lt());
                        out_front += (uint32_t)__popcll(m0);
                        if (key1 == b) pos[1] = out_front + (uint32_t)__popcll(m1 & lanemask_lt());
                        out_front += (uint32_t)__popcll(m1);
                    }
                    for (uint32_t w = 0; w < (two ? 2u : 1u); ++w) {
                        const f3 bo = w ? bo1 : bo0, bd = w ? bd1 : bd0;
                        const uint32_t child_node = w ? child1 : child0;
                        const uint32_t oi = pos[w];
                        if (active && oi + out_back < ps.region + 0u) {
                            const size_t r = base + oi;
                            st4<2>(&out_q[r], make_float4(bo.x, bo.y, bo.z, bd.x));
                            st4<2>(&out_q[ps.qstride + r], make_float4(bd.y, bd.z, __uint_as_float(slot), __uint_as_float(((level + 1u) << 4) | (child_node << 8))));
                        }
                    }
                }
            }
        }
        __builtin_amdgcn_wave_barrier();
        if (out_front + out_back > ps.region) { if (lane == 0) counters->overflow = 1u; out_front = 0u; out_back = 0u; }
        if (out_counts != nullptr && lane == 0) out_counts[chunk] = make_uint2(out_front, out_back);
        out_nrad = out_front; out_nshadow = out_back;
        acc_bounce += out_front; acc_shadow += out_back + ((unsigned long long)skipped << 32); acc_hits += cnt - dropped;
    }
}

__device__ __forceinline__ void flush_shade_counters(DCounters* counters, uint32_t wave, unsigned long long acc_bounce, unsigned long long acc_shadow, unsigned long long acc_hits)
{
    if (lane_id() == 0) {
        DCounters* cs = &counters[wave % kShards];
        if (acc_bounce) atomicAdd(&cs->bounce, acc_bounce);
        if (acc_shadow & 0xFFFFFFFFull) atomicAdd(&cs->shadow, acc_shadow & 0xFFFFFFFFull);
        if (acc_shadow >> 32) atomicAdd(&cs->shadow_skipped, acc_shadow >> 32);
        if (acc_hits & 0xFFFFFFFFull) atomicAdd(&cs->primary_hits, acc_hits & 0xFFFFFFFFull);
        if (acc_hits >> 32) atomicAdd(&cs->primary_culled, acc_hits >> 32);
    }
}

template <bool PRIMARY, bool WALK, bool RASTER = false, bool RAYS = false>
__global__ __launch_bounds__(kBlock, PRIMARY ? (WALK ? kShadePWBlocks : kShadePBlocks) : (WALK ? kShadeSWBlocks : kShadeSBlocks)) void shade_kernel(DScene sc, DCamera cam, DPass ps, uint32_t level,
                                                      const float4* __restrict__ in_q, const uint2* __restrict__ in_counts,
                                                      const float4* __restrict__ hits,
                                                      float4* __restrict__ out_q, uint2* __restrict__ out_counts, uint32_t* cursor,
                                                      float* __restrict__ slot_L, uint32_t* __restrict__ sample_slot,
                                                      const uint32_t* __restrict__ film_n, DCounters* counters)
{
    extern __shared__ uint32_t s_list[];
    const LinearList list{ &s_list[(threadIdx.x >> 6) * ps.list_cap] };
    float4* lds_hits = RASTER ? (float4*)&s_list[kWavesPerBlock * ps.list_cap] + (threadIdx.x >> 6) * ps.chunk : nullptr;
    const uint32_t wave = blockIdx.x * kWavesPerBlock + (threadIdx.x >> 6);
    unsigned long long acc_bounce = 0, acc_shadow = 0, acc_hits = 0, acc_tris = 0;
    PullState pull; uint32_t chunk = 0u;
    while (pull_chunk(cursor, ps.nchunks, pull, chunk, 0u, PRIMARY ? LiveLists() : live_lists(ps))) {
        uint32_t o_rad, o_sh;
        shade_chunk<PRIMARY, LinearList, WALK, RASTER, RAYS>(sc, cam, ps, level, chunk, list, in_q, PRIMARY ? 0u : in_counts[chunk].x, o_rad, o_sh, hits, out_q, out_counts, slot_L, sample_slot, film_n, counters, acc_bounce, acc_shadow, acc_hits,
                                                       lds_hits, (RASTER && (ps.flags & 2u)) ? &acc_tris : nullptr);
        if (PRIMARY && ps.live != nullptr && (o_rad | o_sh) != 0u && lane_id() == 0) {
            const uint32_t k = chunk % kMaxCursors;
            const uint32_t at = atomicAdd(&ps.live_count[(size_t)k * kCursorStride + kLiveCountOffset], 1u);
            ps.live[(size_t)k * ps.live_cap + at] = chunk;
        }
    }
    flush_shade_counters(counters, wave, acc_bounce, acc_shadow, PRIMARY ? acc_hits : 0ull);
    if (RASTER && acc_tris && lane_id() == 0) atomicAdd(&counters[wave % kShards].tris_tested, acc_tris);
}

template <int REC>
__device__ f3 node_radiance(const float* __restrict__ L, const DPass& ps, uint32_t nlights, uint32_t level, uint32_t index)
{
    const uint32_t node = ps.level_first[level] + index;
    f3 rad = mk3(0.0f, 0.0f, 0.0f);
    for (uint32_t li = 0; li < nlights; ++li) {
        const float* p = L + 3ull * ((size_t)node * nlights + li) * ps.nslots;
        rad = add3(rad, mk3(p[0], p[1], p[2]));
    }
    if constexpr (REC == 0) {
        return rad;
    } else {
        const uint32_t k = ps.spread * (uint32_t)REC;
        f3 sum = mk3(0.0f, 0.0f, 0.0f);
        for (uint32_t c = 0; c < k; ++c) sum = add3(sum, node_radiance<REC - 1>(L, ps, nlights, level + 1, index * k + c));
        const f3 sub = vscale(sum, div_rn(1.0f, (float)k));
        return add3(rad, sub);
    }
}

template <uint32_t kResolveLanes, bool DIRECT>
__global__ __launch_bounds__(256) void resolve_kernel(DPass ps, uint32_t width, uint32_t nlights, const float* __restrict__ slot_L,
                                                     const uint32_t* __restrict__ sample_slot,
                                                     float* film_sum, float* film_sumsq, uint32_t* film_n, float* debug_color, uint32_t* ctrl, float* film_direct)
{
    if (ctrl != nullptr && blockIdx.x == 0)
        for (uint32_t i = threadIdx.x; i < kMaxRounds * kMaxCursors * 4u; i += blockDim.x)
            ctrl[(size_t)(i / (kMaxCursors * 4u)) * kCtrlWordsPerRound + (size_t)((i / 4u) % kMaxCursors) * kCursorStride + (i % 4u) * kConfirmCursorOffset] = 0u;
    const uint32_t gid = blockIdx.x * blockDim.x + threadIdx.x;
    const uint32_t j = gid % kResolveLanes;
    const bool live = gid / kResolveLanes < ps.npix;
    const uint32_t p = live ? gid / kResolveLanes : ps.npix - 1u;
    const uint32_t spp = ps.nsamples / ps.npix;
    const uint32_t pixel = ps.use_explicit ? ps.explicit_pixel : pass_pixel(ps, width, p);
    f3 sum = mk3(0, 0, 0), sumsq = mk3(0, 0, 0), direct = mk3(0, 0, 0);
    uint32_t n = 0;
    if (!ps.use_explicit) {
        sum = mk3(film_sum[3ull * pixel], film_sum[3ull * pixel + 1], film_sum[3ull * pixel + 2]);
        sumsq = mk3(film_sumsq[3ull * pixel], film_sumsq[3ull * pixel + 1], film_sumsq[3ull * pixel + 2]);
        n = film_n[pixel];
        if constexpr (DIRECT) direct = mk3(film_direct[3ull * pixel], film_direct[3ull * pixel + 1], film_direct[3ull * pixel + 2]);
    }
    const int group_lane0 = lane_id() & ~(int)(kResolveLanes - 1u);
    const bool dead = ps.block_culled != nullptr && ps.block_culled[(uint32_t)(sample_index(ps, 0u, p) / ps.chunk) % ps.cull_blocks] != 0u;
    const bool on = ps.use_explicit || pixel_active(ps, width, pixel);
    for (uint32_t s0 = 0; s0 < spp; s0 += kResolveLanes) {
        const uint32_t sl = (s0 + j < spp && !dead && on) ? sample_slot[sample_index(ps, s0 + j, p)] : 0xFFFFFFFFu;
        const float* L = slot_L + 3ull * (size_t)sl;
// ... 929 lines not shown
```

### raytracer-rs_amd/csrc/renderer.cpp

```cpp
#include "renderer.hpp"
#include "display.hpp"
#include "lightmap.hpp"
#include <algorithm>
#include <array>
#include <chrono>
#include <cmath>
#include <cstdio>
#include <cstdlib>
#include <cstring>
#include "kernels.hpp"
#include "octree.hpp"

namespace mi355rt {

namespace {
void pcg4d(uint32_t v[4])
{
    for (int i = 0; i < 4; ++i) v[i] = v[i] * 1664525u + 1013904223u;
    v[0] += v[1] * v[3]; v[1] += v[2] * v[0]; v[2] += v[0] * v[1]; v[3] += v[1] * v[2];
    for (int i = 0; i < 4; ++i) v[i] ^= v[i] >> 16;
    v[0] += v[1] * v[3]; v[1] += v[2] * v[0]; v[2] += v[0] * v[1]; v[3] += v[1] * v[2];
}
float u01(uint32_t bits) { return (float)(bits >> 9) * (1.0f / 8388608.0f); }
}

bool Renderer::fail(hipError_t e, const char* what)
{
    last_error = std::string(what) + ": " + hipGetErrorString(e);
    return false;
}
#define HIP_TRY(expr) do { hipError_t e__ = (expr); if (e__ != hipSuccess) return fail(e__, #expr); } while (0)

bool Renderer::bind()
{
    HIP_TRY(hipSetDevice(cfg.device));
    return true;
}

template <class T> bool Renderer::upload(DeviceBuffer<T>& buf, const void* src, size_t bytes)
{
    HIP_TRY(buf.alloc(bytes ? bytes : 16, &hbm_bytes_));
    if (bytes && src) HIP_TRY(hipMemcpy(buf.get(), src, bytes, hipMemcpyHostToDevice));
    else if (bytes) HIP_TRY(hipMemset(buf.get(), 0, bytes));
    return true;
}

template <class T> bool Renderer::upload(T*& dptr, const void* src, size_t bytes)
{
    scene_bufs_.emplace_back();
    if (!upload(scene_bufs_.back(), src, bytes)) return false;
    dptr = static_cast<T*>(scene_bufs_.back().get());
    return true;
}

std::unique_ptr<Renderer> Renderer::create(const SceneData& scene, const mi355rt_config& cfg, std::string& err, int& code)
{
    std::unique_ptr<Renderer> r(new Renderer());
    r->cfg = cfg;
    if (!r->init(scene, err, code)) return nullptr;
    return r;
}

void Renderer::build_sample_table(std::vector<float>& table4)
{
    table.resize((size_t)kNumSamples * 3);
    table4.assign((size_t)kNumSamples * 4, 0.0f);
    for (uint32_t i = 0; i < kNumSamples; ++i) {
        for (uint32_t attempt = 0;; ++attempt) {
            uint32_t h[4] = { i, attempt, 0xFFFFFFFFu, (uint32_t)cfg.seed };
            pcg4d(h);
            Vec3 d(u01(h[0]) * 2.0f + -1.0f, u01(h[1]) * 2.0f + -1.0f, u01(h[2]) * 2.0f + -1.0f);
            if (dot(d, d) < 1.0f) {
                Vec3 nrm = d.normalized();
                table[3 * (size_t)i] = nrm.x; table[3 * (size_t)i + 1] = nrm.y; table[3 * (size_t)i + 2] = nrm.z;
                table4[4 * (size_t)i] = nrm.x; table4[4 * (size_t)i + 1] = nrm.y; table4[4 * (size_t)i + 2] = nrm.z;
                break;
            }
        }
    }
}

bool Renderer::set_seed(uint64_t seed)
{
    if (!bind()) return false;
    if (!settle_speculation()) return false;
// ... 56 lines not shown

    ntri = scene.ntri();
    nlights_ = (uint32_t)scene.lights.size();
    camera = Camera::from_orientation_matrix(cfg.width, cfg.height, Matrix::from_array(scene.cameras[0].orientation), scene.cameras[0].fov_deg);

    const auto t_bvh = std::chrono::steady_clock::now();
    bool on_device = false;
    if (cfg.flags & MI355RT_FLAG_DEVICE_LBVH) {
        std::string why; double ms[2];
        on_device = build_bvh_device(scene.tri_verts.data(), scene.tri_geom.data(), ntri, bvh, why, ms);
        if (on_device) { lbvh_device_ms_ = ms[0]; }
        else last_error = "device LBVH not used (" + why + "): host SAH build instead";
    }
    if (!on_device) build_bvh(scene.tri_verts.data(), scene.tri_geom.data(), ntri, bvh);
    bvh_on_device_ = on_device;
    wide_ = false;
    if (kernels_walk_wide_nodes()) {
        build_wide(bvh);
        if (!bvh.nodes4.empty()) wide_ = true;
        else if (bvh.root >= 0) { err = "this build's kernels walk the 4-wide tree, which does not serve this scene"; code = MI355RT_E_INVALID; return false; }
    }
    build_ms_[0] = std::chrono::duration<double, std::milli>(std::chrono::steady_clock::now() - t_bvh).count();
    collect_cull_boxes();
    if (bvh.max_depth > kBvhMaxDepth) { err = "internal: BVH deeper than the traversal stack"; code = MI355RT_E_INVALID; return false; }
    std::vector<float> normals((size_t)std::max(ntri, 1u) * 4, 0.0f);
    for (uint32_t t = 0; t < ntri; ++t) {
        const float* v = &scene.tri_verts[9 * (size_t)t];
        Vec3 v0(v[0], v[1], v[2]), v1(v[3], v[4], v[5]), v2(v[6], v[7], v[8]);
        Vec3 n = cross(v1 - v0, v2 - v0).normalized();
        normals[4 * (size_t)t] = n.x; normals[4 * (size_t)t + 1] = n.y; normals[4 * (size_t)t + 2] = n.z;
        uint32_t g = scene.tri_geom[t];
        std::memcpy(&normals[4 * (size_t)t + 3], &g, 4);
    }
    std::vector<float> table4;
    build_sample_table(table4);
    void* d_nodes = nullptr; void* d_tris = nullptr; void* d_normals = nullptr; void* d_table = nullptr;
    DMaterial* d_mats = nullptr; DLight* d_lights = nullptr; DTexture* d_tex = nullptr; float* d_texels = nullptr;
    if (wide_ ? !upload(d_nodes, bvh.nodes4.data(), bvh.nodes4.size() * sizeof(BvhNode4)) : !upload(d_nodes, bvh.nodes.data(), bvh.nodes.size() * sizeof(BvhNode))) return bail();
    if (!upload(d_tris, bvh.tris.data(), bvh.tris.size() * sizeof(BvhTri))) return bail();
    if (!upload(d_normals, normals.data(), normals.size() * sizeof(float))) return bail();
    if (!upload(d_table, table4.data(), table4.size() * sizeof(float))) return bail();
    std::vector<DMaterial> mats(std::max<size_t>(scene.materials.size(), 1));
    for (size_t i = 0; i < scene.materials.size(); ++i) {
        const MaterialData& m = scene.materials[i];
        mats[i] = DMaterial{ m.rgb[0], m.rgb[1], m.rgb[2], m.kind == 1 ? (0x80000000u | m.tex_id) : 0u };
    }
    if (!upload(d_mats, mats.data(), mats.size() * sizeof(DMaterial))) return bail();
    std::vector<DLight> lights(std::max<size_t>(scene.lights.size(), 1));
    for (size_t i = 0; i < scene.lights.size(); ++i) {
        const LightData& l = scene.lights[i];
        lights[i] = DLight{ l.pos[0], l.pos[1], l.pos[2], l.color[0], l.color[1], l.color[2], 0.0f, 0.0f };
    }
    float* d_light_maps = nullptr; uint32_t light_map_res = 0;
    if (!scene.lights.empty() && scene.lights.size() <= 8 && ntri > 0 && !getenv("MI355RT_NO_LIGHT_MAP")) {
        const auto t_lm = std::chrono::steady_clock::now();
        double diag2 = 0.0;
        { float mn[3] = { 3e38f, 3e38f, 3e38f }, mx[3] = { -3e38f, -3e38f, -3e38f };
          for (size_t i = 0; i < scene.tri_verts.size(); ++i) { const int a = (int)(i % 3); mn[a] = std::min(mn[a], scene.tri_verts[i]); mx[a] = std::max(mx[a], scene.tri_verts[i]); }
          for (int a = 0; a < 3; ++a) diag2 += ((double)mx[a] - mn[a]) * ((double)mx[a] - mn[a]); }
        const double pad = 2e-4 * std::sqrt(diag2) + 1e-7;
        uint32_t res = 512;
        while (res > 16 && (size_t)6 * res * res * 4 * scene.lights.size() > ((size_t)64 << 20)) res /= 2;
        const uint64_t work_cap = 4ull << 20;
        for (const LightData& l : scene.lights) while (res > 16 && light_map_work(scene.tri_verts.data(), ntri, l.pos, res) > work_cap) res /= 2;
        std::vector<float> all; all.reserve((size_t)6 * res * res * scene.lights.size());
        bool finite = true;
        for (size_t i = 0; i < scene.lights.size() && finite; ++i) {
            const LightData& l = scene.lights[i];
            if (!std::isfinite(l.pos[0]) || !std::isfinite(l.pos[1]) || !std::isfinite(l.pos[2])) { finite = false; break; }
            LightMap lm; build_light_map(scene.tri_verts.data(), ntri, l.pos, pad, res, lm);
            all.insert(all.end(), lm.dist2.begin(), lm.dist2.end());
            const double tail = std::max(lm.nearest - pad, 0.0);
            lights[i].tail2 = std::isfinite(tail) ? (float)std::min(tail * tail * (1.0 - 1e-6), 3.0e38) : 3.0e38f;
            if ((double)lights[i].tail2 > tail * tail) lights[i].tail2 = std::nextafterf(lights[i].tail2, 0.0f);
        }
        if (finite) {
            if (!upload(d_light_maps, all.data(), all.size() * sizeof(float))) return bail();
            light_map_res = res;
        }
        light_map_ms_ = std::chrono::duration<double, std::milli>(std::chrono::steady_clock::now() - t_lm).count();
        if (getenv("MI355RT_DEBUG_CULL")) fprintf(stderr, "[mi355rt] light maps: %zu lights, %u texels per face edge, %.1f ms\n", scene.lights.size(), light_map_res, light_map_ms_);
    }
    if (!upload(d_lights, lights.data(), lights.size() * sizeof(DLight))) return bail();
    std::vector<DTexture> tex(std::max<size_t>(scene.textures.size(), 1));
    std::vector<float> texels;
    for (size_t i = 0; i < scene.textures.size(); ++i) {
        const TextureData& t = scene.textures[i];
        if (t.rgb.size() != (size_t)t.width * t.height * 3 || t.rgb.empty()) { err = "texture size mismatch"; code = MI355RT_E_INVALID; return false; }
        tex[i] = DTexture{ t.width, t.height, texels.size() / 3 };
        texels.insert(texels.end(), t.rgb.begin(), t.rgb.end());
    }
    if (!upload(d_tex, tex.data(), tex.size() * sizeof(DTexture))) return bail();
    if (!upload(d_texels, texels.data(), texels.size() * sizeof(float))) return bail();
    dscene_.nodes = d_nodes; dscene_.tris = d_tris; dscene_.normals = d_normals; dscene_.materials = d_mats;
    dscene_.lights = d_lights; dscene_.textures = d_tex; dscene_.texels = d_texels; dscene_.table = d_table;
    dscene_.root = bvh.root; dscene_.nlights = nlights_; dscene_.ntri = ntri;
    dscene_.light_maps = d_light_maps; dscene_.light_map_res = light_map_res;
    dscene_.oct_nodes = nullptr; dscene_.oct_leaf_tris = nullptr; dscene_.prim_tris = nullptr; dscene_.oct_info = nullptr; dscene_.tri_home = nullptr; dscene_.oct_single_leaf = 0u;
    std::memset(dscene_.oct_root, 0, sizeof dscene_.oct_root);
    mode_ = (cfg.flags & MI355RT_FLAG_OCTREE_SEMANTICS) ? kModeOctreeWalk : (cfg.flags & MI355RT_FLAG_TRUE_CLOSEST_HIT) ? kModeTrueClosest : kModeConfirm;
    if (mode_ != kModeTrueClosest) {
        Octree oct;
        const auto t_oct = std::chrono::steady_clock::now();
        build_octree(scene.tri_verts.data(), ntri, cfg.triangles_per_leaf, oct);
        build_ms_[1] = std::chrono::duration<double, std::milli>(std::chrono::steady_clock::now() - t_oct).count();
        oct_stats_[0] = (uint32_t)oct.nodes.size(); oct_stats_[1] = oct.inner; oct_stats_[2] = oct.leaves;
        oct_stats_[3] = oct.empty_leaves; oct_stats_[4] = oct.max_depth; oct_stats_[5] = (uint32_t)oct.leaf_tris.size();
        std::vector<BvhTri> prim_tris(std::max(ntri, 1u));
        std::memset(prim_tris.data(), 0, prim_tris.size() * sizeof(BvhTri));
        for (uint32_t t = 0; t < ntri; ++t) {
            const float* v = &scene.tri_verts[9 * (size_t)t];
            for (int a = 0; a < 3; ++a) { prim_tris[t].v0[a] = v[a]; prim_tris[t].e1[a] = v[3 + a] - v[a]; prim_tris[t].e2[a] = v[6 + a] - v[a]; }
            prim_tris[t].prim = t; prim_tris[t].geom = scene.tri_geom[t];
        }
        void* d_oct = nullptr; uint32_t* d_leaf = nullptr; void* d_ptris = nullptr;
        if (!upload(d_oct, oct.nodes.data(), oct.nodes.size() * sizeof(OctNodeFlat))) return bail();
        if (!upload(d_leaf, oct.leaf_tris.data(), oct.leaf_tris.size() * 4)) return bail();
        if (!upload(d_ptris, prim_tris.data(), prim_tris.size() * sizeof(BvhTri))) return bail();
        dscene_.oct_nodes = d_oct; dscene_.oct_leaf_tris = d_leaf; dscene_.prim_tris = d_ptris;
        std::vector<int2> info(oct.nodes.size());
        std::vector<uint32_t> home(std::max(ntri, 1u), 0xFFFFFFFEu);
        for (size_t i = 0; i < oct.nodes.size(); ++i) {
            const OctNodeFlat& f = oct.nodes[i];
            if (f.first_child >= 0) { info[i].x = f.first_child; info[i].y = 0; continue; }
            info[i].x = ~(int32_t)f.tri_first; info[i].y = (int32_t)f.tri_count;
            for (uint32_t k = 0; k < f.tri_count; ++k) {
                uint32_t& h = home[oct.leaf_tris[f.tri_first + k]];
                h = h == 0xFFFFFFFEu ? (uint32_t)i : 0xFFFFFFFFu;
            }
        }
        int2* d_info = nullptr; uint32_t* d_home = nullptr;
        if (!upload(d_info, info.data(), info.size() * sizeof(int2))) return bail();
        if (!upload(d_home, home.data(), home.size() * 4)) return bail();
        dscene_.oct_info = d_info; dscene_.tri_home = d_home;
        dscene_.oct_single_leaf = (mode_ == kModeConfirm && oct.nodes.size() == 1) ? 1u : 0u;
        for (int a = 0; a < 3; ++a) { dscene_.oct_root[a] = oct.nodes[0].cmin[a]; dscene_.oct_root[3 + a] = oct.nodes[0].cmax[a]; }
    }

    const size_t npix = (size_t)cfg.width * cfg.height;
    if (!upload(d_film_sum_, nullptr, npix * 12) || !upload(d_film_sumsq_, nullptr, npix * 12) || !upload(d_film_n_, nullptr, npix * 4)) return bail();
    if ((cfg.flags & MI355RT_FLAG_DIRECT_FILM) && !upload(d_film_direct_, nullptr, npix * 12)) return bail();
    if (!upload(d_ldr_, nullptr, npix * 4)) return bail();
    ldr_dirty_.assign(cfg.height, (uint8_t)1);
    if (hipEventCreateWithFlags(&ev_tonemap_, hipEventDisableTiming) != hipSuccess || hipEventCreateWithFlags(&ev_gather_, hipEventDisableTiming) != hipSuccess) { err = "hipEventCreate failed"; return false; }
    if (hipEventCreateWithFlags(&ev_call_done_, hipEventDisableTiming) != hipSuccess || hipEventCreateWithFlags(&ev_spec_done_, hipEventDisableTiming) != hipSuccess
        || hipStreamCreateWithFlags(&read_stream_, hipStreamNonBlocking) != hipSuccess) { err = "hipEventCreate / hipStreamCreate failed"; return false; }
    std::vector<uint32_t> all(cfg.height);
    for (uint32_t r = 0; r < cfg.height; ++r) {
        all[r] = r;
        if ((r / cfg.stripe_rows) % cfg.stripe_world == cfg.stripe_rank) owned_rows.push_back(r);
    }
    if (!upload(d_all_rows_, all.data(), all.size() * 4)) return bail();
    if (!upload(d_owned_rows_, owned_rows.data(), owned_rows.size() * 4)) return bail();
    if (!upload(d_tmp_rows_, nullptr, 64 * 4)) return bail();
    if (!upload(d_counters_, nullptr, sizeof(DCounters) * kShards)) return bail();
    if (h_counters_.alloc(sizeof(DCounters) * kShards) != hipSuccess) { err = "pinned host allocation failed"; return false; }
    std::memset(h_counters_.get(), 0, sizeof(DCounters) * kShards);
    slices_[0].stream = stream_;
    for (uint32_t i = 0; i < kMaxSlices; ++i) {
        if (i && hipStreamCreateWithFlags(&slices_[i].stream, hipStreamNonBlocking) != hipSuccess) { err = "hipStreamCreate failed"; return false; }
        if (hipEventCreateWithFlags(&slices_[i].done, hipEventDisableTiming) != hipSuccess) { err = "hipEventCreate failed"; return false; }
        if (!upload(slices_[i].d_ctrl, nullptr, kMaxRounds * kCtrlWordsPerRound * 4)) return bail();
        if (!upload(slices_[i].d_rows, nullptr, (size_t)cfg.height * 4)) return bail();
    }
    if (const char* e = getenv("MI355RT_SLICES")) { int v = atoi(e); if (v >= 1 && v <= (int)kMaxSlices) slices = (uint32_t)v; }
    if (!upload(d_debug_color_, nullptr, 16)) return bail();

    records_per_sample_ = 1;
    for (uint32_t l = 0; l <= cfg.recursions; ++l) {
        uint32_t nl = level_first[l + 1] - level_first[l];
        uint32_t nn = l < cfg.recursions ? level_first[l + 2] - level_first[l + 1] : 0;
        records_per_sample_ = std::max(records_per_sample_, nl * std::max(nlights_, 1u) + nn);
    }
    max_level_nodes_ = 1;
    for (uint32_t l = 0; l <= cfg.recursions; ++l) max_level_nodes_ = std::max(max_level_nodes_, level_first[l + 1] - level_first[l]);
    code = MI355RT_OK;
    return true;
}

Renderer::~Renderer()
// ... 386 lines not shown
    const bool confirm_here = mode_ == kModeConfirm && !dscene_.oct_single_leaf;
    for (uint32_t r = 0; r < cfg.recursions + 2; ++r) {
        const bool fuse_primary = r == 0 && cam.tile_ofs != nullptr && mode_ != kModeOctreeWalk;
        const void* in_q = r == 0 ? nullptr : sl.d_queue[(r - 1) & 1].get();
        const void* in_c = r == 0 ? nullptr : sl.d_chunk_counts[(r - 1) & 1].get();
        const bool balance_dbg = !fuse_primary && count && getenv("MI355RT_DEBUG_UTIL") && mode_ != kModeOctreeWalk;
        if (!fuse_primary) {
            if (timed) {
                if (ev_used_ + 2 > ev_pool_.size()) {
                    for (int k = 0; k < 2; ++k) { hipEvent_t ev; HIP_TRY(hipEventCreate(&ev)); ev_pool_.push_back(ev); }
                }
                HIP_TRY(hipEventRecord(ev_pool_[ev_used_], st));
                ev_secondary_.resize(ev_pool_.size() / 2); ev_secondary_[ev_used_ / 2] = r > 0;
            }
            if (balance_dbg) {
                DCounters init{};
                HIP_TRY(hipMemcpy(&init, d_counters_.get(), sizeof init, hipMemcpyDeviceToHost));
                init.t_first_end = ~0ull; init.t_start = ~0ull; init.t_last_end = 0; init.t_sum_end = 0; init.n_waves = 0;
                HIP_TRY(hipMemcpy(d_counters_.get(), &init, sizeof init, hipMemcpyHostToDevice));
            }
            if (mode_ == kModeOctreeWalk)
                HIP_TRY(launch_trace_octree(st, num_cus_, r == 0, dscene_, cam, ps, in_q, in_c, sl.d_hits.get(), sl.d_slot_L.get(), d_film_n_.get(), rays && r == 0));
            else
                HIP_TRY(launch_trace(st, num_cus_, r == 0, count, mode_ == kModeConfirm, dscene_, cam, ps, in_q, in_c, sl.d_hits.get(), sl.d_ctrl.get() + r * kCtrlWordsPerRound, sl.d_slot_L.get(), d_film_n_.get(), d_counters_.get(), rays && r == 0));
            if (timed) { HIP_TRY(hipEventRecord(ev_pool_[ev_used_ + 1], st)); ev_used_ += 2; }
            ++launches_;
        }
        const bool shade_walks = confirm_here && r <= cfg.recursions;
        if (confirm_here && r != 0)
            HIP_TRY(launch_confirm(st, num_cus_, false, shade_walks, dscene_, cam, ps, in_q, in_c, sl.d_hits.get(), sl.d_ctrl.get() + r * kCtrlWordsPerRound + kConfirmCursorOffset, sl.d_slot_L.get(), d_film_n_.get()));
        if (balance_dbg) {
            DCounters c0{};
            HIP_TRY(hipStreamSynchronize(st));
            HIP_TRY(hipMemcpy(&c0, d_counters_.get(), sizeof c0, hipMemcpyDeviceToHost));
            {
                DCounters sh[kShards], t{};
                HIP_TRY(hipMemcpy(sh, d_counters_.get(), sizeof sh, hipMemcpyDeviceToHost));
                for (const DCounters& x : sh) { t.lanes_inner += x.lanes_inner; t.lanes_leaf += x.lanes_leaf; t.lanes_done += x.lanes_done; t.lane_samples += x.lane_samples;
                                                t.refills += x.refills; t.refill_passes += x.refill_passes; t.refill_rays += x.refill_rays; t.inner_execs += x.inner_execs; t.leaf_execs += x.leaf_execs; }
                static DCounters prev{};
                if (t.lane_samples < prev.lane_samples) prev = DCounters{};
                const double it = (double)(t.lane_samples - prev.lane_samples);
                if (it > 0)
                    fprintf(stderr, "[mi355rt] trace round %u census: iterations %.0f, lanes at inner %.1f / at leaf %.1f / idle-or-finished %.1f per iteration; inner execs %.2f, leaf execs %.2f per iteration; refills %llu, passes %llu, rays per refill %.1f\n",
                            r, it, (t.lanes_inner - prev.lanes_inner) / it, (t.lanes_leaf - prev.lanes_leaf) / it, (t.lanes_done - prev.lanes_done) / it,
                            (t.inner_execs - prev.inner_execs) / it, (t.leaf_execs - prev.leaf_execs) / it,
                            t.refills - prev.refills, t.refill_passes - prev.refill_passes, (double)(t.refill_rays - prev.refill_rays) / std::max<double>(1.0, (double)(t.refills - prev.refills)));
                prev = t;
            }
            if (c0.n_waves)
                fprintf(stderr, "[mi355rt] trace round %u: %llu waves, mean wave busy %.1f us, first wave out of work at %.1f us, last at %.1f us\n", r, c0.n_waves,
                        (double)c0.t_sum_end / c0.n_waves / 100.0, (double)(c0.t_first_end - c0.t_start) / 100.0, (double)(c0.t_last_end - c0.t_start) / 100.0);
        }
        if (r <= cfg.recursions)
            HIP_TRY(launch_shade(st, num_cus_, r == 0, shade_walks, dscene_, cam, ps, r, in_q, in_c, sl.d_hits.get(), sl.d_queue[r & 1].get(), sl.d_chunk_counts[r & 1].get(), sl.d_ctrl.get() + r * kCtrlWordsPerRound + kShadeCursorOffset, sl.d_slot_L.get(), sl.d_sample_slot.get(), d_film_n_.get(), d_counters_.get(), fuse_primary, rays && r == 0));
    }
    if (free_rays) HIP_TRY(launch_resolve_rays(st, ps, nlights_, sl.d_slot_L.get(), sl.d_sample_slot.get(), feed->rgb, feed->direct, feed->tuv, feed->prim, sl.d_ctrl.get()));
    else HIP_TRY(launch_resolve(st, ps, cfg.width, nlights_, sl.d_slot_L.get(), sl.d_sample_slot.get(), d_film_sum_.get(), d_film_sumsq_.get(), d_film_n_.get(), d_film_direct_.get(), d_debug_color_.get(), sl.d_ctrl.get()));
    sl.ctrl_clean = true;
    return true;
}

bool Renderer::begin_call()
{
    if (!bind()) return false;
    if (!settle_speculation()) return false;
    call_done_valid_ = false;
    ev_used_ = 0; launches_ = 0;
    counts_pending_ = false;
    HIP_TRY(hipMemsetAsync(d_counters_.get(), 0, sizeof(DCounters) * kShards, stream_));
    HIP_TRY(hipEventRecord(ev_begin_, stream_));
    active_slices_ = 1;
    return true;
}

bool Renderer::fetch_counts(uint64_t primary, bool timed_call)
{
    DCounters c{};
    const DCounters* shard = h_counters_.get();
    for (uint32_t i = 0; i < kShards; ++i) {
        const DCounters& s = shard[i];
        c.bounce += s.bounce; c.shadow += s.shadow; c.primary_hits += s.primary_hits;
        c.nodes_visited += s.nodes_visited; c.tris_tested += s.tris_tested; c.overflow |= s.overflow;
        c.inner_execs += s.inner_execs; c.leaf_execs += s.leaf_execs; c.primary_culled += s.primary_culled; c.shadow_skipped += s.shadow_skipped;
        c.t_sum_cycles += s.t_sum_cycles; c.t_sum_real += s.t_sum_real;
        for (int k = 0; k < 6; ++k) c.visits_below[k] += s.visits_below[k];
    }
    counts = mi355rt_ray_counts{};
    counts.primary = primary; counts.bounce = c.bounce; counts.shadow = c.shadow + c.shadow_skipped; counts.primary_hits = c.primary_hits;
    counts.shadow_skipped = c.shadow_skipped;
    counts.nodes_visited = c.nodes_visited; counts.tris_tested = c.tris_tested; counts.trace_launches = launches_;
    counts.inner_execs = c.inner_execs; counts.leaf_execs = c.leaf_execs; counts.primary_culled = c.primary_culled;
    if (getenv("MI355RT_DEBUG_UTIL") && c.nodes_visited)
        fprintf(stderr, "[mi355rt] inner-node visits with node index < 64 / 128 / 256 / 512 / 1024 / 2048: %.3f / %.3f / %.3f / %.3f / %.3f / %.3f of %llu\n", (double)c.visits_below[0] / c.nodes_visited, (double)c.visits_below[1] / c.nodes_visited,
                (double)c.visits_below[2] / c.nodes_visited, (double)c.visits_below[3] / c.nodes_visited, (double)c.visits_below[4] / c.nodes_visited, (double)c.visits_below[5] / c.nodes_visited, c.nodes_visited);
    if (getenv("MI355RT_DEBUG_UTIL")) fprintf(stderr, "[mi355rt] inner execs %llu (lane util %.3f) leaf execs %llu (lane util %.3f)\n", c.inner_execs, c.inner_execs ? (double)c.nodes_visited / (64.0 * c.inner_execs) : 0.0, c.leaf_execs, c.leaf_execs ? (double)c.tris_tested / (64.0 * c.leaf_execs) : 0.0);
    if (timed_call) {
        float ms = 0.0f;
        HIP_TRY(hipEventElapsedTime(&ms, ev_begin_, ev_end_));
        counts.total_ms = ms;
    }
    double tms = 0.0, sms = 0.0; uint64_t nsec = 0;
    for (size_t i = 0; i + 1 < ev_used_; i += 2) {
        float t = 0.0f;
        HIP_TRY(hipEventElapsedTime(&t, ev_pool_[i], ev_pool_[i + 1]));
        tms += t;
        if (i / 2 < ev_secondary_.size() && ev_secondary_[i / 2]) { sms += t; ++nsec; }
    }
    counts.trace_ms = tms; counts.trace_secondary_ms = sms; counts.trace_secondary_launches = nsec;
    counts.shader_clock_mhz = c.t_sum_real ? (double)c.t_sum_cycles / (double)c.t_sum_real * 100.0 : 0.0;
    if (c.overflow) { last_error = (c.overflow & 2u) ? "internal: traversal stack overflow (instrumented build: a ray held more deferred nodes than the stack has rows)" : "internal: ray queue overflow"; return false; }
    return true;
}

bool Renderer::queue_counts_copy()
{
    HIP_TRY(hipMemcpyAsync(h_counters_.get(), d_counters_.get(), sizeof(DCounters) * kShards, hipMemcpyDeviceToHost, stream_));
    return true;
}

bool Renderer::join_slices()
{
    for (uint32_t i = 1; i < active_slices_; ++i) {
        HIP_TRY(hipEventRecord(slices_[i].done, slices_[i].stream));
        HIP_TRY(hipStreamWaitEvent(stream_, slices_[i].done, 0));
    }
    active_slices_ = 1;
    return true;
}

bool Renderer::end_call(uint64_t primary, bool wait)
{
    if (!join_slices()) return false;
    HIP_TRY(hipEventRecord(ev_end_, stream_));
    if (!queue_counts_copy()) return false;
    if (!wait) { counts_pending_ = true; pending_primary_ = primary; pending_timed_ = true; return true; }
    HIP_TRY(hipStreamSynchronize(stream_));
    return fetch_counts(primary, true);
}

bool Renderer::last_counts(mi355rt_ray_counts& out)
{
    if (counts_pending_) {
        if (!bind()) return false;
        if (call_done_valid_) HIP_TRY(hipEventSynchronize(ev_call_done_));
        else HIP_TRY(hipStreamSynchronize(stream_));
        counts_pending_ = false;
        const bool timed = pending_timed_; pending_timed_ = false;
        if (!fetch_counts(pending_primary_, timed)) return false;
    }
    out = counts;
    return true;
}

struct FrameWindow { uint32_t first = 0, total = 0, next_row = 0; };
static FrameWindow frame_window(uint32_t current_row, uint32_t height, uint32_t stripe_rows, uint32_t world, uint32_t rank, const std::vector<uint32_t>& owned)
{
    FrameWindow w;
    uint32_t row = current_row;
    bool have_first = false;
    for (int k = 0; k < 50; ++k) {
        if ((row / stripe_rows) % world == rank) {
            if (!have_first) { w.first = (uint32_t)(std::lower_bound(owned.begin(), owned.end(), row) - owned.begin()); have_first = true; }
            ++w.total;
        }
        row = (row + 1) % height;
    }
    w.next_row = row;
    return w;
}

void Renderer::mark_dirty_window(uint32_t first, uint32_t total)
{
// ... 731 lines not shown
```

### raytracer-rs_amd/csrc/renderer.hpp

```cpp
#pragma once
#include <hip/hip_runtime_api.h>
#include <array>
#include <memory>
#include <string>
#include <vector>
#include "../../include/mi355rt.h"
#include "bvh.hpp"
#include "camera.hpp"
#include "device_buffer.hpp"
#include "device_types.hpp"
#include "scene.hpp"

namespace mi355rt {

class Renderer {
public:
    static std::unique_ptr<Renderer> create(const SceneData& scene, const mi355rt_config& cfg, std::string& err, int& code);
    ~Renderer();

    uint32_t trace_frame_additive();
    bool render(uint32_t spp, bool wait = true);
    bool render_adaptive(const mi355rt_adaptive_config& ac, mi355rt_adaptive_stats& st);
    bool adaptive_tile_mask(const mi355rt_adaptive_config& ac, uint8_t* out, uint32_t& active);
    uint32_t tiles_x() const { return (cfg.width + kAdaptiveTile - 1) / kAdaptiveTile; }
    uint32_t tiles_y() const { return (cfg.height + kAdaptiveTile - 1) / kAdaptiveTile; }
    bool get_tonemapped(uint32_t* out, size_t n);
    bool tonemap_owned_rows_device(uint32_t* device_out, size_t n, hipStream_t caller_stream = nullptr);
    bool last_counts(mi355rt_ray_counts& out);
    bool film_get(float* sum, float* sumsq, uint32_t* n);
    bool film_get_direct(float* sum);
    bool set_seed(uint64_t seed);
    bool set_flags(uint32_t flags);
    bool film_clear();
    struct FilmPlanes { const float* sum; const float* sumsq; const uint32_t* n; const float* direct; };
    bool film_put(const FilmPlanes& in, bool add);
    bool intersect(const float* rays6, size_t n, float* tuv, uint32_t* prim, uint8_t* blocked);
    bool trace_rays(const float* rays6, const uint32_t* keys2, size_t n, bool device, const mi355rt_ray_outputs& out);
    bool render_rays(const float* rays6, uint32_t spp, bool device);
    bool caller_ray_film() const { return caller_ray_film_; }
    bool synchronize();
    uint32_t slot_rows() const;
    uint32_t rows_of_rank(uint32_t rank) const;
    bool gather_prepare(bool root);
    uint32_t* gather_slot(uint32_t rank) { return d_gather_ ? d_gather_.get() + (gather_is_root_ ? (size_t)rank : 0) * slot_rows() * cfg.width : nullptr; }
    bool tonemap_to_gather_slot();
    bool finish_gather(uint32_t* host_out, size_t n);
    hipStream_t stream() const { return stream_; }
    hipEvent_t gather_event() const { return ev_gather_; }
    bool comm_available();
    bool comm_init(const uint8_t* id128);
    bool comm_gather(uint32_t root, uint32_t* host_out, size_t n);
    void comm_destroy();
    uint32_t comm_ranks();
    long check_guards();
    size_t hbm_allocated_bytes() const { return hbm_bytes_; }
    bool debug_gather_rate(uint32_t table_nodes, uint32_t steps, double out[3]);
    bool debug_slab(const float* inv_rays6, const float* cubes6, size_t n, uint8_t* hit, float* tmin);
    bool film_stat(bool variances, float* rgb);
    bool get_guides(float* depth, float* normal3, float* albedo3, uint32_t* prim);
    bool get_denoised(const mi355rt_denoise_config& dc, float* rgb, uint32_t* packed, bool split = false);
    bool has_direct_film() const { return (cfg.flags & MI355RT_FLAG_DIRECT_FILM) != 0; }
    bool display_histogram(uint32_t source, const mi355rt_denoise_config& dn, mi355rt_luminance_histogram& out);
    bool get_display(const mi355rt_display_config& dc, const mi355rt_denoise_config& dn, uint32_t* packed, float& exposure_used);
    void speculation_stats(uint64_t out[2]) const { out[0] = spec_launched_; out[1] = spec_adopted_; }
    bool debug_numerics(const float* a, const float* b, size_t n, float* q, float* r, float* p);
    bool debug_sample(uint32_t pixel, uint32_t sampleno, float* color3, float* node_L, size_t nodes);

    Camera camera;
    mi355rt_config cfg;
    mi355rt_ray_counts counts{};
    std::string last_error;
    std::vector<float> table;
    std::vector<uint32_t> owned_rows;
    Bvh bvh;
    uint32_t ntri = 0;
    uint32_t current_row = 0;
    uint32_t slices = 1;
    bool slices_explicit = false;
    uint32_t nodes_per_sample = 1;
    uint32_t level_first[kMaxLevels + 1] = { 0 };
    std::vector<std::array<float, 6>> cull_boxes_;
    size_t hbm_bytes_ = 0;
    DeviceBuffer<uint32_t> d_cull_mask_;
    std::vector<float> mask_key_;
    float mask_dom_[4] = { 0, 0, 0, 0 };
    bool mask_valid_ = false;
    DeviceBuffer<uint2> d_tile_ofs_, d_tile_entries_;
    std::vector<float> bins_key_;
    uint32_t bins_layout_[3] = { 0, 0, 0 };
    bool bins_valid_ = false;
    double bins_ms_ = 0.0; size_t bins_entries_ = 0;
    uint32_t oct_stats_[8] = { 0 };
    double build_ms_[2] = { 0.0, 0.0 };
    double light_map_ms_ = 0.0;
    bool bvh_on_device_ = false;
    bool wide_ = false;
    uint32_t traversal_rows() const { return (wide_ ? bvh.stack_need4 : bvh.max_depth) + 1u; }
    double lbvh_device_ms_ = 0.0;
    enum Mode { kModeConfirm = 0, kModeOctreeWalk = 1, kModeTrueClosest = 2 };
    Mode mode_ = kModeConfirm;

private:
    Renderer() = default;
    bool init(const SceneData& scene, std::string& err, int& code);
    bool bind();
    bool fail(hipError_t e, const char* what);
    struct Slice {
        hipStream_t stream = nullptr;
        hipEvent_t done = nullptr;
        std::vector<uint32_t> rows;
        DeviceBuffer<uint32_t> d_rows;
        DeviceBuffer<uint32_t> d_ctrl;
        bool ctrl_clean = true;
        DeviceBuffer<> d_queue[2];
        DeviceBuffer<uint32_t> d_chunk_counts[2];
        DeviceBuffer<> d_hits;
        DeviceBuffer<uint32_t> d_hit_prim;
        DeviceBuffer<float> d_slot_L;
        DeviceBuffer<> d_slot_ps;
        DeviceBuffer<uint32_t> d_sample_slot;
        DeviceBuffer<uint32_t> d_live;
        DeviceBuffer<uint32_t> d_block_culled;
        std::vector<float> cull_key;
        size_t capacity = 0;
        size_t queue_records = 0;
        size_t count_entries = 0;
        template <class F> void for_each_pass_buffer(F f) { f(d_queue[0]); f(d_queue[1]); f(d_chunk_counts[0]); f(d_chunk_counts[1]); f(d_hits); f(d_hit_prim); f(d_slot_L); f(d_slot_ps); f(d_sample_slot); f(d_live); }
        void release_pass_buffers() { for_each_pass_buffer([](auto& b) { b.reset(); }); capacity = 0; }
    };
    bool ensure_pass_capacity(Slice& sl, size_t nsamples);
    void free_pass_buffers();
    bool assign_slice_rows(uint32_t nslices);
    struct RayFeed { uint32_t mode; const float* rays; const uint32_t* keys; uint32_t base; uint32_t count; float4* hit; float* rgb; float* direct; float* tuv; uint32_t* prim; };
    bool run_pass(Slice& sl, const uint32_t* d_rows, uint32_t row0, uint32_t nrows, uint32_t spp, bool explicit_sample, uint32_t epixel, uint32_t esample, uint32_t row_wrap = 0xFFFFFFFFu,
                  const uint8_t* tile_active = nullptr, const RayFeed* feed = nullptr);
    bool enqueue_frame(uint32_t spp, hipEvent_t fork, const uint8_t* tile_active, const RayFeed* feed = nullptr);
    bool caller_ray_film_ = false;
    bool join_slices();
    bool adaptive_verdict(const mi355rt_adaptive_config& ac, uint32_t& tiles, uint64_t& pixels);
    DeviceBuffer<uint8_t> d_tile_active_;
    DeviceBuffer<unsigned long long> d_tile_count_;
    bool refresh_guides();
    DeviceBuffer<float4> d_guide0_, d_guide1_;
    std::vector<float> guides_key_;
    DeviceBuffer<float4> d_dn_ping_, d_dn_pong_;
    DeviceBuffer<uint32_t> d_dn_flags_, d_dn_packed_;
    DeviceBuffer<float> d_dn_rgb_;
    bool run_denoise(const mi355rt_denoise_config& dc, bool rgb, bool packed, bool split);
    bool display_source(uint32_t source, const mi355rt_denoise_config& dn, const float*& img, bool& film);
    bool display_hist_queue(const float* img, bool film, mi355rt_luminance_histogram& out);
    DeviceBuffer<uint32_t> d_disp_hist_, d_disp_packed_;
    DeviceBuffer<float> d_disp_table_;
    void describe_pass(DPass& ps, const Slice& sl, const uint32_t* d_rows, uint32_t row0, uint32_t row_wrap, uint32_t npix, size_t nsamples, uint32_t chunk,
                       bool explicit_sample, uint32_t epixel, uint32_t esample) const;
    bool begin_call();
    bool end_call(uint64_t primary, bool wait = true);
    bool fetch_counts(uint64_t primary, bool timed_call);
    bool queue_counts_copy();
    void mark_dirty_window(uint32_t first, uint32_t total);
    DCamera device_camera(const DPass* layout = nullptr, const std::vector<uint32_t>* rows = nullptr);
    bool refresh_tile_bins(DCamera& c, const double inv[3][3], double pad, double zmin, const DPass& ps, const std::vector<uint32_t>& rows);
    bool refresh_cull_mask(DCamera& c, const double inv[3][3], double pad, double zmin, bool build);
    bool project_triangles(const DCamera& c, const double inv[3][3], double pad, double zmin);
    struct TriRect { double x0, x1, y0, y1; };
    std::vector<TriRect> tri_rects_;
    std::vector<float> rects_key_;
    bool rects_ok_ = false;
    void collect_cull_boxes();
    void build_sample_table(std::vector<float>& table4);
    template <class T> bool upload(DeviceBuffer<T>& buf, const void* src, size_t bytes);
    template <class T> bool upload(T*& dptr, const void* src, size_t bytes);

    int num_cus_ = 0;
    hipStream_t stream_ = nullptr;
    hipEvent_t ev_begin_ = nullptr, ev_end_ = nullptr;
    std::vector<hipEvent_t> ev_pool_;
    size_t ev_used_ = 0;
// ... 46 lines not shown
```

Baseline: 18530.

## Skip bounce rays proven to escape via per-triangle reflection direction masks

Builds, on the host at scene load, a per-triangle bitmask over cube-map direction bins that marks which outgoing directions could hit other geometry. Bounce rays whose direction falls in a clear bin, and whose origin passes a plane guard, are dropped before enqueueing, since they are proven to miss everything. This removes traversal work for escaping secondary rays, at the cost of a multi-threaded precomputation, extra device memory and a mask lookup per bounce. Skipped rays are still counted as bounce rays in the reported totals.

```diff
diff --git a/include/mi355rt.h b/include/mi355rt.h
--- a/include/mi355rt.h
+++ b/include/mi355rt.h
@@ -88,6 +88,7 @@
     uint64_t trace_secondary_launches;
     double shader_clock_mhz;
     uint64_t shadow_skipped;
+    uint64_t bounce_skipped;
 } mi355rt_ray_counts;
 
 void mi355rt_default_config(mi355rt_config* cfg);
@@ -225,10 +226,13 @@
 uint32_t mi355rt_tree_nodes(const mi355rt_handle* h);
 int mi355rt_debug_speculation(const mi355rt_handle* h, uint64_t out[2]);
 int mi355rt_debug_light_map(const float* tri_verts, uint32_t ntri, const float light[3], double pad, uint32_t res, float* out_dist2, double* nearest);
+int mi355rt_debug_reflect_mask(const float* tri_verts, uint32_t ntri, double pad, uint32_t bins, uint64_t work_budget, uint32_t* out_words, double info[8]);
 
 int mi355rt_debug_wide_bvh(const float* tri_verts, uint32_t ntri, uint32_t out[8]);
 
 int mi355rt_accel_stats(const mi355rt_handle* h, uint32_t out[8]);
+int mi355rt_reflect_mask_info(const mi355rt_handle* h, double out[4]);
+int mi355rt_debug_rays_read(const mi355rt_handle* h, uint64_t* out);
 int mi355rt_bvh_build_info(const mi355rt_handle* h, uint32_t out[2]);
 int mi355rt_octree_stats(const mi355rt_handle* h, uint32_t out[8]);
 uint32_t mi355rt_device_count(const mi355rt_handle* h);
diff --git a/raytracer-rs_amd/__init__.py b/raytracer-rs_amd/__init__.py
--- a/raytracer-rs_amd/__init__.py
+++ b/raytracer-rs_amd/__init__.py
@@ -63,12 +63,13 @@
         ("trace_ms", C.c_double), ("total_ms", C.c_double),
         ("trace_secondary_ms", C.c_double), ("trace_secondary_launches", C.c_uint64), ("shader_clock_mhz", C.c_double),
         ("shadow_skipped", C.c_uint64),
+        ("bounce_skipped", C.c_uint64),
     ]
 
     def as_dict(self):
         d = {name: getattr(self, name) for name, _ in self._fields_}
         d["total_rays"] = self.primary + self.bounce + self.shadow
-        d["traced_rays"] = d["total_rays"] - self.primary_culled - self.shadow_skipped
+        d["traced_rays"] = d["total_rays"] - self.primary_culled - self.shadow_skipped - self.bounce_skipped
         return d
 
 
@@ -190,6 +191,9 @@
     ("mi355rt_tree_nodes", C.c_uint32, [_H]),
     ("mi355rt_debug_speculation", C.c_int, [_H, C.POINTER(C.c_uint64)]),
     ("mi355rt_debug_light_map", C.c_int, [_F, C.c_uint32, _F, C.c_double, C.c_uint32, _F, C.POINTER(C.c_double)]),
+    ("mi355rt_debug_reflect_mask", C.c_int, [_F, C.c_uint32, C.c_double, C.c_uint32, C.c_uint64, _U, C.POINTER(C.c_double)]),
+    ("mi355rt_reflect_mask_info", C.c_int, [_H, C.POINTER(C.c_double)]),
+    ("mi355rt_debug_rays_read", C.c_int, [_H, C.POINTER(C.c_uint64)]),
     ("mi355rt_debug_wide_bvh", C.c_int, [_F, C.c_uint32, _U]),
     ("mi355rt_accel_stats", C.c_int, [_H, _U]),
     ("mi355rt_octree_stats", C.c_int, [_H, _U]),
@@ -643,6 +647,16 @@
         self._check(lib().mi355rt_accel_stats(self._h, _up(out)))
         return dict(nodes=int(out[0]), leaves=int(out[1]), max_depth=int(out[2]), max_leaf=int(out[3]),
                     node_bytes=int(out[4]), tri_bytes=int(out[5]), bvh_build_ms=int(out[6]) / 1000.0, octree_build_ms=int(out[7]) / 1000.0)
+
+    def reflect_mask_info(self):
+        out = (C.c_double * 4)()
+        self._check(lib().mi355rt_reflect_mask_info(self._h, out))
+        return dict(bins=int(out[0]), build_ms=float(out[1]), clear_share=float(out[2]), bytes=int(out[3]))
+
+    def debug_rays_read(self):
+        out = C.c_uint64(0)
+        self._check(lib().mi355rt_debug_rays_read(self._h, C.byref(out)))
+        return int(out.value)
 
     def bvh_build_info(self):
         out = np.zeros(2, np.uint32)
@@ -743,6 +757,20 @@
     return out, nearest.value
 
 
+def debug_reflect_mask(tri_verts, pad, bins=8, work_budget=0, min_cos=0.0, pad_angle=0.0):
+    v = np.ascontiguousarray(tri_verts, np.float32).reshape(-1, 9)
+    info = (C.c_double * 8)()
+    info[4], info[5] = float(min_cos), float(pad_angle)
+    stride = 6 * bins * bins // 32 + 4
+    out = np.zeros((v.shape[0], stride), np.uint32)
+    code = lib().mi355rt_debug_reflect_mask(_fp(v), v.shape[0], float(pad), int(bins), int(work_budget), _up(out), info)
+    if code != 0:
+        raise RuntimeError("mi355rt_debug_reflect_mask failed: %d" % code)
+    d = dict(stride=int(info[0]), build_ms=float(info[1]), work=int(info[2]), clear_bits=int(info[3]), min_cos=float(info[4]), pad_angle=float(info[5]),
+             bary_margin=float(info[6]), built=bool(info[7]))
+    return (out if d["built"] else None), d
+
+
 def debug_wide_bvh(tri_verts):
     v = np.ascontiguousarray(tri_verts, np.float32).reshape(-1, 9)
     out = (C.c_uint32 * 8)()
diff --git a/raytracer-rs_amd/csrc/capi.cpp b/raytracer-rs_amd/csrc/capi.cpp
--- a/raytracer-rs_amd/csrc/capi.cpp
+++ b/raytracer-rs_amd/csrc/capi.cpp
@@ -6,6 +6,7 @@
 #include <vector>
 #include "display.hpp"
 #include "lightmap.hpp"
+#include "reflmask.hpp"
 #include "../../include/mi355rt.h"
 #include "group.hpp"
 #include "renderer.hpp"
@@ -650,6 +651,17 @@
     mi355rt::build_light_map(tri_verts, ntri, light, pad, res, lm);
     std::memcpy(out_dist2, lm.dist2.data(), lm.dist2.size() * sizeof(float));
     if (nearest) *nearest = lm.nearest;
+    return MI355RT_OK;
+}
+int mi355rt_debug_reflect_mask(const float* tri_verts, uint32_t ntri, double pad, uint32_t bins, uint64_t work_budget, uint32_t* out_words, double info[8])
+{
+    if ((ntri && !tri_verts) || !info || !(pad >= 0.0)) return MI355RT_E_INVALID;
+    mi355rt::ReflMask m;
+    const double min_cos = info[4] > 0.0 ? info[4] : mi355rt::kReflMinCos, pad_angle = info[5] > 0.0 ? info[5] : mi355rt::kReflPadAngle;
+    const bool built = ntri != 0 && mi355rt::build_reflect_mask(tri_verts, ntri, pad, bins, work_budget ? work_budget : ~0ull, m, min_cos, pad_angle);
+    info[0] = (double)mi355rt::refl_mask_stride(bins); info[1] = m.build_ms; info[2] = (double)m.work; info[3] = (double)m.clear_bits;
+    info[4] = min_cos; info[5] = pad_angle; info[6] = (double)mi355rt::kReflBary; info[7] = built ? 1.0 : 0.0;
+    if (built && out_words) std::memcpy(out_words, m.words.data(), m.words.size() * sizeof(uint32_t));
     return MI355RT_OK;
 }
 
@@ -734,6 +746,18 @@
     out[0] = h->r->bvh_on_device_ ? 1u : 0u; out[1] = (uint32_t)(h->r->lbvh_device_ms_ * 1000.0);
     return MI355RT_OK;
 }
+int mi355rt_debug_rays_read(const mi355rt_handle* h, uint64_t* out)
+{
+    if (!h || !out) return MI355RT_E_INVALID;
+    *out = h->r->rays_read_;
+    return MI355RT_OK;
+}
+int mi355rt_reflect_mask_info(const mi355rt_handle* h, double out[4])
+{
+    if (!h || !out) return MI355RT_E_INVALID;
+    std::memcpy(out, h->r->reflect_mask_info_, sizeof h->r->reflect_mask_info_);
+    return MI355RT_OK;
+}
 int mi355rt_octree_stats(const mi355rt_handle* h, uint32_t out[8])
 {
     if (!h || !out) return MI355RT_E_INVALID;
diff --git a/raytracer-rs_amd/csrc/device_types.hpp b/raytracer-rs_amd/csrc/device_types.hpp
--- a/raytracer-rs_amd/csrc/device_types.hpp
+++ b/raytracer-rs_amd/csrc/device_types.hpp
@@ -41,6 +41,8 @@
     const uint32_t* tri_home;
     const float* light_maps;
     uint32_t light_map_res;
+    const uint32_t* refl_mask;
+    uint32_t refl_bins, refl_stride;
     int32_t root;
     uint32_t nlights;
     uint32_t ntri;
@@ -133,6 +135,7 @@
     unsigned long long t_sum_cycles, t_sum_real;
     unsigned long long visits_below[6];
     unsigned long long refills, refill_passes, refill_rays;
+    unsigned long long bounce_skipped;
 };
 
 }
diff --git a/raytracer-rs_amd/csrc/group.cpp b/raytracer-rs_amd/csrc/group.cpp
--- a/raytracer-rs_amd/csrc/group.cpp
+++ b/raytracer-rs_amd/csrc/group.cpp
@@ -66,7 +66,7 @@
     for (size_t i = 0; i < devs_.size(); ++i) {
         if (!ok[i]) return fail_from(i);
         const mi355rt_ray_counts& c = devs_[i]->counts;
-        counts_.primary += c.primary; counts_.bounce += c.bounce; counts_.shadow += c.shadow; counts_.shadow_skipped += c.shadow_skipped; counts_.primary_hits += c.primary_hits;
+        counts_.primary += c.primary; counts_.bounce += c.bounce; counts_.shadow += c.shadow; counts_.shadow_skipped += c.shadow_skipped; counts_.bounce_skipped += c.bounce_skipped; counts_.primary_hits += c.primary_hits;
         counts_.primary_culled += c.primary_culled; counts_.nodes_visited += c.nodes_visited; counts_.tris_tested += c.tris_tested;
         counts_.trace_launches += c.trace_launches; counts_.inner_execs += c.inner_execs; counts_.leaf_execs += c.leaf_execs;
         counts_.trace_ms += c.trace_ms; counts_.total_ms = std::max(counts_.total_ms, c.total_ms);
@@ -85,7 +85,7 @@
     for (size_t i = 0; i < devs_.size(); ++i) {
         mi355rt_ray_counts c{};
         if (!devs_[i]->last_counts(c)) return fail_from(i);
-        out.primary += c.primary; out.bounce += c.bounce; out.shadow += c.shadow; out.shadow_skipped += c.shadow_skipped; out.primary_hits += c.primary_hits;
+        out.primary += c.primary; out.bounce += c.bounce; out.shadow += c.shadow; out.shadow_skipped += c.shadow_skipped; out.bounce_skipped += c.bounce_skipped; out.primary_hits += c.primary_hits;
         out.primary_culled += c.primary_culled; out.nodes_visited += c.nodes_visited; out.tris_tested += c.tris_tested;
         out.trace_launches += c.trace_launches; out.inner_execs += c.inner_execs; out.leaf_execs += c.leaf_execs;
         out.trace_ms += c.trace_ms; out.total_ms = std::max(out.total_ms, c.total_ms);
diff --git a/raytracer-rs_amd/csrc/kernels.hip b/raytracer-rs_amd/csrc/kernels.hip
--- a/raytracer-rs_amd/csrc/kernels.hip
+++ b/raytracer-rs_amd/csrc/kernels.hip
@@ -8,6 +8,7 @@
 #include "device_math.hpp"
 #include "device_types.hpp"
 #include "kernels.hpp"
+#include "reflmask.hpp"
 #include "traverse.hpp"
 
 namespace mi355rt {
@@ -679,6 +680,31 @@
     return (l2 * 0.98011f < bound) & (l2 * 1.0002e-4f < lt.tail2);
 }
 
+__device__ __forceinline__ uint32_t reflection_record(const DScene& sc, const float4 h)
+{
+    if (sc.refl_mask == nullptr || !((h.y > kReflBary) & (h.z > kReflBary) & (h.y + h.z < 1.0f - kReflBary))) return kMiss;
+    return __float_as_uint(h.w) * sc.refl_stride;
+}
+__device__ __forceinline__ bool reflection_proves_miss(const DScene& sc, uint32_t rec_first, const f3 n, const f3 bo, const f3 bd)
+{
+    if (rec_first == kMiss) return false;
+    const float ax = fabsf(bd.x), ay = fabsf(bd.y), az = fabsf(bd.z);
+    uint32_t m; float vm, va, vb;
+    if (ax >= ay && ax >= az) { m = 0u; vm = bd.x; va = bd.y; vb = bd.z; }
+    else if (ay >= az) { m = 1u; vm = bd.y; va = bd.x; vb = bd.z; }
+    else { m = 2u; vm = bd.z; va = bd.x; vb = bd.y; }
+    const float am = fabsf(vm);
+    if (!(am > 0.0f)) return false;
+    const uint32_t B = sc.refl_bins;
+    const float fB = (float)B, u = div_rn(va, am), v = div_rn(vb, am);
+    const int i = min(max((int)((u * 0.5f + 0.5f) * fB), 0), (int)B - 1), j = min(max((int)((v * 0.5f + 0.5f) * fB), 0), (int)B - 1);
+    const uint32_t bit = ((2u * m + (vm < 0.0f ? 1u : 0u)) * B + (uint32_t)i) * B + (uint32_t)j;
+    const uint32_t* __restrict__ rec = sc.refl_mask + rec_first;
+    if ((rec[bit >> 5] >> (bit & 31u)) & 1u) return false;
+    const float4 g = *(const float4*)(rec + (sc.refl_stride - kReflGuardWords));
+    return dot3(sub3(bo, mk3(g.x, g.y, g.z)), n) > g.w;
+}
+
 template <bool PRIMARY, class List, bool WALK = false, bool RASTER = false, bool RAYS = false>
 __device__ __forceinline__ void shade_chunk(const DScene& sc, const DCamera& cam, const DPass& ps, uint32_t level, uint32_t chunk, const List list,
                                             const float4* __restrict__ in_q, uint32_t in_nrad, uint32_t& out_nrad, uint32_t& out_nshadow,
@@ -729,12 +755,12 @@
             }
         }
         __builtin_amdgcn_wave_barrier();
-        uint32_t out_front = 0u, out_back = 0u, dropped = 0u, skipped = 0u;
+        uint32_t out_front = 0u, out_back = 0u, dropped = 0u, skipped = 0u, bskipped = 0u;
         for (uint32_t j = 0; j < cnt; j += 64u) {
             bool active = j + (uint32_t)lane < cnt;
             const bool in_batch = active;
             f3 o = mk3(0, 0, 0), d = mk3(0, 0, 1), hp = mk3(0, 0, 0), n = mk3(0, 0, 1);
-            uint32_t slot = 0u, node = 0u, pixel = 0u, sampleno = 0u, geom = 0u;
+            uint32_t slot = 0u, node = 0u, pixel = 0u, sampleno = 0u, geom = 0u, refl_rec = kMiss;
             float4 h = make_float4(0, 0, 0, 0);
             if (active) {
                 const uint32_t i = list[j + (uint32_t)lane];
@@ -764,6 +790,7 @@
                 const float4 nn = ((const float4*)sc.normals)[__float_as_uint(h.w)];
                 n = mk3(nn.x, nn.y, nn.z);
                 geom = __float_as_uint(nn.w);
+                if (level < ps.recursions) refl_rec = reflection_record(sc, h);
             }
             for (uint32_t li = 0; li < sc.nlights; ++li) {
                 bool want = false, is_free = false;
@@ -822,8 +849,14 @@
                         bd0 = mk3(tv0.x, tv0.y, tv0.z); bo0 = add3(hp, sscale(0.00001f, bd0));
                         bd1 = mk3(tv1.x, tv1.y, tv1.z); bo1 = add3(hp, sscale(0.00001f, bd1));
                     }
+                    bool make0 = active, make1 = active && two;
+                    if (sc.refl_mask != nullptr) {
+                        if (make0) make0 = !reflection_proves_miss(sc, refl_rec, n, bo0, bd0);
+                        if (make1) make1 = !reflection_proves_miss(sc, refl_rec, n, bo1, bd1);
+                        bskipped += (uint32_t)__popcll(__ballot(active && !make0)) + (uint32_t)__popcll(__ballot(active && two && !make1));
+                    }
                     uint32_t pos[2] = { 0u, 0u };
-                    const uint32_t key0 = active ? dir_bin(bd0) : kSortBins, key1 = (active && two) ? dir_bin(bd1) : kSortBins;
+                    const uint32_t key0 = make0 ? dir_bin(bd0) : kSortBins, key1 = make1 ? dir_bin(bd1) : kSortBins;
                     for (uint32_t b = 0; b < kSortBins; ++b) {
                         const unsigned long long m0 = __ballot(key0 == b), m1 = __ballot(key1 == b);
                         if (key0 == b) pos[0] = out_front + (uint32_t)__popcll(m0 & lanemask_lt());
@@ -835,7 +868,7 @@
                         const f3 bo = w ? bo1 : bo0, bd = w ? bd1 : bd0;
                         const uint32_t child_node = w ? child1 : child0;
                         const uint32_t oi = pos[w];
-                        if (active && oi + out_back < ps.region + 0u) {
+                        if ((w ? make1 : make0) && oi + out_back < ps.region + 0u) {
                             const size_t r = base + oi;
                             st4<2>(&out_q[r], make_float4(bo.x, bo.y, bo.z, bd.x));
                             st4<2>(&out_q[ps.qstride + r], make_float4(bd.y, bd.z, __uint_as_float(slot), __uint_as_float(((level + 1u) << 4) | (child_node << 8))));
@@ -848,7 +881,7 @@
         if (out_front + out_back > ps.region) { if (lane == 0) counters->overflow = 1u; out_front = 0u; out_back = 0u; }
         if (out_counts != nullptr && lane == 0) out_counts[chunk] = make_uint2(out_front, out_back);
         out_nrad = out_front; out_nshadow = out_back;
-        acc_bounce += out_front; acc_shadow += out_back + ((unsigned long long)skipped << 32); acc_hits += cnt - dropped;
+        acc_bounce += out_front + ((unsigned long long)bskipped << 32); acc_shadow += out_back + ((unsigned long long)skipped << 32); acc_hits += cnt - dropped;
     }
 }
 
@@ -856,7 +889,8 @@
 {
     if (lane_id() == 0) {
         DCounters* cs = &counters[wave % kShards];
-        if (acc_bounce) atomicAdd(&cs->bounce, acc_bounce);
+        if (acc_bounce & 0xFFFFFFFFull) atomicAdd(&cs->bounce, acc_bounce & 0xFFFFFFFFull);
+        if (acc_bounce >> 32) atomicAdd(&cs->bounce_skipped, acc_bounce >> 32);
         if (acc_shadow & 0xFFFFFFFFull) atomicAdd(&cs->shadow, acc_shadow & 0xFFFFFFFFull);
         if (acc_shadow >> 32) atomicAdd(&cs->shadow_skipped, acc_shadow >> 32);
         if (acc_hits & 0xFFFFFFFFull) atomicAdd(&cs->primary_hits, acc_hits & 0xFFFFFFFFull);
diff --git a/raytracer-rs_amd/csrc/reflmask.cpp b/raytracer-rs_amd/csrc/reflmask.cpp
--- /dev/null
+++ b/raytracer-rs_amd/csrc/reflmask.cpp
@@ -0,0 +1,334 @@
+#include "reflmask.hpp"
+#include <algorithm>
+#include <atomic>
+#include <chrono>
+#include <cmath>
+#include <cstring>
+#include <limits>
+#include <thread>
+
+namespace mi355rt {
+namespace {
+
+struct V3 { double x, y, z; };
+inline V3 sub(V3 a, V3 b) { return { a.x - b.x, a.y - b.y, a.z - b.z }; }
+inline V3 add(V3 a, V3 b) { return { a.x + b.x, a.y + b.y, a.z + b.z }; }
+inline V3 mul(V3 a, double s) { return { a.x * s, a.y * s, a.z * s }; }
+inline double dot(V3 a, V3 b) { return a.x * b.x + a.y * b.y + a.z * b.z; }
+inline V3 cross(V3 a, V3 b) { return { a.y * b.z - a.z * b.y, a.z * b.x - a.x * b.z, a.x * b.y - a.y * b.x }; }
+inline double len(V3 a) { return std::sqrt(dot(a, a)); }
+inline bool unit(V3& a) { const double l = len(a); if (!(l > 0.0) || !std::isfinite(l)) return false; a = mul(a, 1.0 / l); return true; }
+
+const int kAxisA[3] = { 1, 0, 0 }, kAxisB[3] = { 2, 2, 1 };
+
+struct Bin {
+    V3 corner[4];
+    V3 face[4];
+    V3 centre;
+    double cos_rho, sin_rho;
+};
+
+void make_bins(uint32_t B, std::vector<Bin>& bins)
+{
+    bins.resize((size_t)6 * B * B);
+    for (uint32_t f = 0; f < 6; ++f) {
+        const int m = (int)(f >> 1), a = kAxisA[m], b = kAxisB[m];
+        const double sg = (f & 1u) ? -1.0 : 1.0;
+        auto dir = [&](double u, double v) { double w[3]; w[m] = sg; w[a] = u; w[b] = v; V3 d = { w[0], w[1], w[2] }; unit(d); return d; };
+        for (uint32_t i = 0; i < B; ++i) for (uint32_t j = 0; j < B; ++j) {
+            Bin& bn = bins[((size_t)f * B + i) * B + j];
+            const double u0 = 2.0 * i / B - 1.0, u1 = 2.0 * (i + 1) / B - 1.0, v0 = 2.0 * j / B - 1.0, v1 = 2.0 * (j + 1) / B - 1.0;
+            bn.corner[0] = dir(u0, v0); bn.corner[1] = dir(u1, v0); bn.corner[2] = dir(u1, v1); bn.corner[3] = dir(u0, v1);
+            bn.centre = dir(0.5 * (u0 + u1), 0.5 * (v0 + v1));
+            double cmin = 1.0;
+            for (int k = 0; k < 4; ++k) {
+                cmin = std::min(cmin, dot(bn.centre, bn.corner[k]));
+                V3 w = cross(bn.corner[k], bn.corner[(k + 1) & 3]); unit(w);
+                if (dot(w, bn.centre) < 0.0) w = mul(w, -1.0);
+                bn.face[k] = w;
+            }
+            cmin = std::max(cmin - 1e-12, -1.0);
+            bn.cos_rho = cmin; bn.sin_rho = std::sqrt(std::max(0.0, 1.0 - cmin * cmin));
+        }
+    }
+}
+
+struct Node { V3 c, h; double r; int32_t left, right; uint32_t first, count; };
+
+struct Tree {
+    std::vector<Node> nodes;
+    std::vector<uint32_t> order;
+    const float* verts;
+    int32_t build(uint32_t lo, uint32_t hi)
+    {
+        V3 mn = { 1e300, 1e300, 1e300 }, mx = { -1e300, -1e300, -1e300 }, cmn = mn, cmx = mx;
+        for (uint32_t k = lo; k < hi; ++k) {
+            const float* v = verts + 9 * (size_t)order[k];
+            V3 c = { 0, 0, 0 };
+            for (int q = 0; q < 3; ++q) {
+                const V3 p = { v[3 * q], v[3 * q + 1], v[3 * q + 2] };
+                mn = { std::min(mn.x, p.x), std::min(mn.y, p.y), std::min(mn.z, p.z) }; mx = { std::max(mx.x, p.x), std::max(mx.y, p.y), std::max(mx.z, p.z) };
+                c = add(c, mul(p, 1.0 / 3.0));
+            }
+            cmn = { std::min(cmn.x, c.x), std::min(cmn.y, c.y), std::min(cmn.z, c.z) }; cmx = { std::max(cmx.x, c.x), std::max(cmx.y, c.y), std::max(cmx.z, c.z) };
+        }
+        const int32_t id = (int32_t)nodes.size();
+        nodes.push_back(Node{});
+        Node nd; nd.c = mul(add(mn, mx), 0.5); nd.h = mul(sub(mx, mn), 0.5); nd.r = len(nd.h) * (1.0 + 1e-12); nd.left = nd.right = -1; nd.first = lo; nd.count = hi - lo;
+        if (hi - lo > 4u) {
+            const V3 e = sub(cmx, cmn);
+            const int ax = e.x >= e.y && e.x >= e.z ? 0 : e.y >= e.z ? 1 : 2;
+            const uint32_t mid = lo + (hi - lo) / 2u;
+            const float* vv = verts;
+            std::nth_element(order.begin() + lo, order.begin() + mid, order.begin() + hi, [vv, ax](uint32_t p, uint32_t q) {
+                const float* a = vv + 9 * (size_t)p; const float* b = vv + 9 * (size_t)q;
+                return (double)a[ax] + a[3 + ax] + a[6 + ax] < (double)b[ax] + b[3 + ax] + b[6 + ax]; });
+            nd.left = build(lo, mid); nd.right = build(mid, hi);
+        }
+        nodes[(size_t)id] = nd;
+        return id;
+    }
+};
+
+struct Walker {
+    const std::vector<Bin>& bins;
+    const std::vector<Bin>& groups;
+    uint32_t B;
+    const Tree& tree;
+    const float* verts;
+    double pad, min_cos, pad_angle, sin_pad;
+    uint32_t nbits;
+    struct Cap { V3 centre; double cos_rho, sin_rho; };
+    std::vector<Cap> bcap, gcap;
+    std::vector<uint16_t> clear[24];
+    uint32_t nclear = 0;
+    V3 normal = { 0, 0, 1 };
+    double up_sin;
+    std::vector<uint16_t> touched, cand;
+    uint64_t work = 0, exacts = 0;
+
+    Walker(const std::vector<Bin>& b, const std::vector<Bin>& g, uint32_t B_, const Tree& t, const float* v, double p, double mc, double pa)
+        : bins(b), groups(g), B(B_), tree(t), verts(v), pad(p), min_cos(mc), pad_angle(pa), sin_pad(std::sin(pa)), nbits((uint32_t)b.size()), up_sin(std::sqrt(1.0 - mc * mc))
+    {
+        for (const Bin& x : b) bcap.push_back(Cap{ x.centre, x.cos_rho, x.sin_rho });
+        for (const Bin& x : g) gcap.push_back(Cap{ x.centre, x.cos_rho, x.sin_rho });
+    }
+    uint32_t group_of(uint32_t b) const { const uint32_t j = b % B, i = (b / B) % B, f = b / (B * B); return f * 4u + (i >= B / 2u ? 2u : 0u) + (j >= B / 2u ? 1u : 0u); }
+
+    static V3 vert(const float* v, int q) { return { v[3 * q], v[3 * q + 1], v[3 * q + 2] }; }
+
+    void cap_touch(V3 d, double cos_half, double sin_half)
+    {
+        touched.clear();
+        {
+            const double c = cos_half * min_cos - sin_half * up_sin, s = sin_half * min_cos + cos_half * up_sin;
+            if (s > 0.0 && dot(normal, d) < c) return;
+        }
+        auto touches = [&](const Cap& bn) {
+            const double c = cos_half * bn.cos_rho - sin_half * bn.sin_rho, s = sin_half * bn.cos_rho + cos_half * bn.sin_rho;
+            return s <= 0.0 || dot(bn.centre, d) >= c;
+        };
+        for (uint32_t g = 0; g < 24u; ++g) {
+            if (clear[g].empty() || !touches(gcap[g])) continue;
+            for (uint16_t b : clear[g]) if (touches(bcap[b])) touched.push_back(b);
+        }
+    }
+    void all_clear() { touched.clear(); for (uint32_t g = 0; g < 24u; ++g) touched.insert(touched.end(), clear[g].begin(), clear[g].end()); }
+    void set_bins(const std::vector<uint16_t>& which, uint32_t* row)
+    {
+        for (uint16_t b : which) {
+            row[b >> 5] |= 1u << (b & 31u);
+            std::vector<uint16_t>& cl = clear[group_of(b)];
+            auto it = std::find(cl.begin(), cl.end(), b);
+            if (it != cl.end()) { *it = cl.back(); cl.pop_back(); --nclear; }
+        }
+    }
+
+    void exact(const V3 tp[3], V3 n, const float* u9, uint32_t* row)
+    {
+        ++work;
+        {
+            bool below = true;
+            for (int i = 0; i < 3 && below; ++i) for (int j = 0; j < 3; ++j) {
+                const V3 d = sub(vert(u9, j), tp[i]);
+                const double nd = dot(n, d);
+                if (!(nd <= 0.0) && !(nd * nd <= 1e-18 * dot(d, d))) { below = false; break; }
+            }
+            if (below) return;
+        }
+        ++exacts;
+        V3 a[9];
+        bool ok = true;
+        for (int i = 0; i < 3 && ok; ++i) for (int j = 0; j < 3; ++j) {
+            V3 d = sub(vert(u9, j), tp[i]);
+            if (!unit(d)) { ok = false; break; }
+            a[3 * i + j] = d;
+        }
+        {
+            V3 mean = { 0, 0, 0 };
+            for (int k = 0; k < 9 && ok; ++k) mean = add(mean, a[k]);
+            double cmin = 1.0;
+            if (ok && unit(mean)) for (int k = 0; k < 9; ++k) cmin = std::min(cmin, dot(mean, a[k])); else cmin = 0.0;
+            if (cmin > 0.1) {
+                cmin -= 1e-12;
+                const double smax = std::sqrt(std::max(0.0, 1.0 - cmin * cmin)), cp = std::cos(pad_angle);
+                cap_touch(mean, cmin * cp - smax * sin_pad, smax * cp + cmin * sin_pad);
+                if (touched.empty()) return;
+            } else all_clear();
+        }
+        cand.assign(touched.begin(), touched.end());
+        touched.clear();
+        for (uint16_t b : cand) {
+            const Bin& bn = bins[b];
+            bool separated = false;
+            for (int f = 0; f < 4 && ok && !separated; ++f) {
+                bool out = true;
+                for (int k = 0; k < 9; ++k) if (!(dot(bn.face[f], a[k]) < -sin_pad - 1e-9)) { out = false; break; }
+                separated = out;
+            }
+            if (!separated) touched.push_back(b);
+        }
+        if (touched.empty()) return;
+        if (ok) {
+            V3 sup[40]; int nsup = 0;
+            for (int p = 0; p < 9 && nsup < 38; ++p) for (int q = p + 1; q < 9 && nsup < 38; ++q) {
+                V3 w = cross(a[p], a[q]);
+                if (!(len(w) > 1e-9) || !unit(w)) continue;
+                double lo = 0.0, hi = 0.0;
+                for (int k = 0; k < 9 && (hi <= 1e-9 || lo >= -1e-9); ++k) { const double s = dot(w, a[k]); lo = std::min(lo, s); hi = std::max(hi, s); }
+                if (hi <= 1e-9) sup[nsup++] = w;
+                else if (lo >= -1e-9) sup[nsup++] = mul(w, -1.0);
+            }
+            cand.assign(touched.begin(), touched.end());
+            touched.clear();
+            for (uint16_t b : cand) {
+                const Bin& bn = bins[b];
+                bool separated = false;
+                for (int s = 0; s < nsup && !separated; ++s) {
+                    bool in = true;
+                    for (int k = 0; k < 4; ++k) if (!(dot(sup[s], bn.corner[k]) > sin_pad + 1e-9)) { in = false; break; }
+                    separated = in;
+                }
+                if (!separated) touched.push_back(b);
+            }
+        }
+        cand.assign(touched.begin(), touched.end());
+        set_bins(cand, row);
+    }
+
+    void triangle(uint32_t t, uint32_t* row, uint32_t stride)
+    {
+        const uint32_t mask_words = stride - kReflGuardWords;
+        for (uint32_t k = 0; k < mask_words; ++k) row[k] = 0xFFFFFFFFu;
+        const float* v = verts + 9 * (size_t)t;
+        std::memcpy(&row[mask_words], v, 12);
+        float hmin = std::numeric_limits<float>::infinity();
+        std::memcpy(&row[mask_words + 3], &hmin, 4);
+        for (int k = 0; k < 9; ++k) if (!std::isfinite(v[k])) return;
+        const V3 p0 = vert(v, 0), p1 = vert(v, 1), p2 = vert(v, 2);
+        V3 n = cross(sub(p1, p0), sub(p2, p0));
+        const double area2 = len(n);
+        const double emax = std::max(len(sub(p1, p0)), std::max(len(sub(p2, p0)), len(sub(p2, p1))));
+        if (!(emax > 0.0) || !unit(n)) return;
+        const double hgt = area2 / emax;
+        if (!(hgt > 1e-3 * emax)) return;
+        double amax = 0.0;
+        for (int k = 0; k < 9; ++k) amax = std::max(amax, std::fabs((double)v[k]));
+        const double slop = 4.0 * std::ldexp(amax, -23) / min_cos;
+        const double bm = 0.5 * (double)kReflBary;
+        if (!(slop < 0.5 * bm * hgt)) return;
+        const V3 tp[3] = { add(mul(p0, 1.0 - 2.0 * bm), mul(add(p1, p2), bm)), add(mul(p1, 1.0 - 2.0 * bm), mul(add(p0, p2), bm)), add(mul(p2, 1.0 - 2.0 * bm), mul(add(p0, p1), bm)) };
+        const V3 ct = mul(add(p0, add(p1, p2)), 1.0 / 3.0);
+        const double rt = std::max(len(sub(tp[0], ct)), std::max(len(sub(tp[1], ct)), len(sub(tp[2], ct))));
+        for (uint32_t g = 0; g < 24u; ++g) clear[g].clear();
+        nclear = 0; normal = n;
+        for (uint32_t b = 0; b < nbits; ++b) {
+            bool up = true;
+            for (int k = 0; k < 4; ++k) if (!(dot(n, bins[b].corner[k]) >= min_cos + 2.0 * pad_angle)) { up = false; break; }
+            if (up) { clear[group_of(b)].push_back((uint16_t)b); ++nclear; row[b >> 5] &= ~(1u << (b & 31u)); }
+        }
+        hmin = (float)(kReflHeightUlps * std::ldexp(emax, -24) * (emax / hgt));
+        if (!(hmin > 0.0f)) return;
+        std::memcpy(&row[mask_words + 3], &hmin, 4);
+        int32_t stack[128]; int sp = 0;
+        stack[sp++] = 0;
+        while (sp > 0 && nclear != 0u) {
+            const Node& nd = tree.nodes[(size_t)stack[--sp]];
+            ++work;
+            const V3 rel = sub(nd.c, p0);
+            if (dot(n, rel) + std::fabs(n.x) * nd.h.x + std::fabs(n.y) * nd.h.y + std::fabs(n.z) * nd.h.z <= 0.0) continue;
+            V3 d = sub(nd.c, ct);
+            const double dist = len(d), R = nd.r + rt + pad;
+            bool far = false;
+            if (dist > R * 1.0000001 && unit(d)) {
+                const double s0 = R / dist, c0 = std::sqrt(std::max(0.0, 1.0 - s0 * s0));
+                const double cp = std::cos(pad_angle), sp_ = sin_pad;
+                const double ch = c0 * cp - s0 * sp_, sh = s0 * cp + c0 * sp_;
+                cap_touch(d, ch, sh);
+                if (touched.empty()) continue;
+                far = s0 < 0.12;
+            }
+            if (far) {
+                cand.assign(touched.begin(), touched.end());
+                set_bins(cand, row);
+            } else if (nd.left < 0) {
+                for (uint32_t k = 0; k < nd.count && nclear != 0u; ++k) {
+                    const uint32_t u = tree.order[nd.first + k];
+                    if (u != t) exact(tp, n, verts + 9 * (size_t)u, row);
+                }
+            } else if (sp + 2 <= 128) {
+                const Node& l = tree.nodes[(size_t)nd.left]; const Node& r = tree.nodes[(size_t)nd.right];
+                const bool l_near = len(sub(l.c, ct)) <= len(sub(r.c, ct));
+                stack[sp++] = l_near ? nd.right : nd.left; stack[sp++] = l_near ? nd.left : nd.right;
+            } else {
+                all_clear();
+                cand.assign(touched.begin(), touched.end());
+                set_bins(cand, row);
+            }
+        }
+    }
+};
+
+}
+
+bool build_reflect_mask(const float* tri_verts, uint32_t ntri, double pad, uint32_t B, uint64_t work_budget, ReflMask& out, double min_cos, double pad_angle)
+{
+    out = ReflMask{};
+    if (ntri == 0 || B < 4 || B > 16 || (6u * B * B) % 128u != 0u || !(pad >= 0.0) || !(min_cos > 0.0 && min_cos < 1.0) || !(pad_angle >= 0.0 && pad_angle < 0.1)) return false;
+    const auto t0 = std::chrono::steady_clock::now();
+    const uint32_t stride = refl_mask_stride(B);
+    std::vector<Bin> bins, groups; make_bins(B, bins); make_bins(2, groups);
+    Tree tree; tree.verts = tri_verts; tree.order.resize(ntri);
+    for (uint32_t i = 0; i < ntri; ++i) tree.order[i] = i;
+    tree.nodes.reserve((size_t)ntri);
+    tree.build(0, ntri);
+    std::vector<uint32_t> words((size_t)ntri * stride);
+    std::atomic<uint32_t> next{ 0 };
+    std::atomic<uint64_t> work{ 0 }, exacts{ 0 };
+    std::atomic<bool> over{ false };
+    auto worker = [&]() {
+        Walker w(bins, groups, B, tree, tri_verts, pad, min_cos, pad_angle);
+        for (;;) {
+            const uint32_t first = next.fetch_add(64u);
+            if (first >= ntri || over.load()) break;
+            for (uint32_t t = first; t < std::min(first + 64u, ntri); ++t) w.triangle(t, &words[(size_t)t * stride], stride);
+            if (work.fetch_add(w.work) + w.work > work_budget) over.store(true);
+            w.work = 0;
+            exacts.fetch_add(w.exacts); w.exacts = 0;
+        }
+    };
+    const uint32_t nthreads = std::max(1u, std::min({ 16u, std::thread::hardware_concurrency(), (ntri + 255u) / 256u }));
+    std::vector<std::thread> pool;
+    for (uint32_t i = 1; i < nthreads; ++i) pool.emplace_back(worker);
+    worker();
+    for (std::thread& th : pool) th.join();
+    out.work = work.load(); out.exact_tests = exacts.load();
+    out.build_ms = std::chrono::duration<double, std::milli>(std::chrono::steady_clock::now() - t0).count();
+    if (over.load()) return false;
+    uint64_t clear_bits = 0;
+    for (uint32_t t = 0; t < ntri; ++t) for (uint32_t k = 0; k < stride - kReflGuardWords; ++k) clear_bits += 32u - (uint32_t)__builtin_popcount(words[(size_t)t * stride + k]);
+    out.bins = B; out.stride = stride; out.words.swap(words); out.clear_bits = clear_bits;
+    return true;
+}
+
+}
diff --git a/raytracer-rs_amd/csrc/reflmask.hpp b/raytracer-rs_amd/csrc/reflmask.hpp
--- /dev/null
+++ b/raytracer-rs_amd/csrc/reflmask.hpp
@@ -0,0 +1,29 @@
+#pragma once
+#include <cstdint>
+#include <vector>
+
+namespace mi355rt {
+
+constexpr double kReflMinCos = 0.05;
+constexpr double kReflPadAngle = 1e-3;
+constexpr float kReflBary = 0.02f;
+constexpr double kReflHeightUlps = 16.0;
+constexpr uint32_t kReflBins = 8;
+constexpr uint32_t kReflGuardWords = 4;
+
+struct ReflMask {
+    uint32_t bins = 0;
+    uint32_t stride = 0;
+    std::vector<uint32_t> words;
+    double build_ms = 0.0;
+    uint64_t work = 0;
+    uint64_t exact_tests = 0;
+    uint64_t clear_bits = 0;
+};
+
+inline uint32_t refl_mask_stride(uint32_t bins) { return 6u * bins * bins / 32u + kReflGuardWords; }
+
+bool build_reflect_mask(const float* tri_verts, uint32_t ntri, double pad, uint32_t bins, uint64_t work_budget, ReflMask& out,
+                        double min_cos = kReflMinCos, double pad_angle = kReflPadAngle);
+
+}
diff --git a/raytracer-rs_amd/csrc/renderer.cpp b/raytracer-rs_amd/csrc/renderer.cpp
--- a/raytracer-rs_amd/csrc/renderer.cpp
+++ b/raytracer-rs_amd/csrc/renderer.cpp
@@ -1,6 +1,7 @@
 #include "renderer.hpp"
 #include "display.hpp"
 #include "lightmap.hpp"
+#include "reflmask.hpp"
 #include <algorithm>
 #include <array>
 #include <chrono>
@@ -223,6 +224,24 @@
         if (getenv("MI355RT_DEBUG_CULL")) fprintf(stderr, "[mi355rt] light maps: %zu lights, %u texels per face edge, %.1f ms\n", scene.lights.size(), light_map_res, light_map_ms_);
     }
     if (!upload(d_lights, lights.data(), lights.size() * sizeof(DLight))) return bail();
+    uint32_t* d_refl_mask = nullptr; uint32_t refl_bins = 0, refl_stride = 0;
+    if (ntri > 0 && cfg.recursions > 0 && !getenv("MI355RT_NO_REFLECT_MASK")) {
+        double diag2 = 0.0;
+        { float mn[3] = { 3e38f, 3e38f, 3e38f }, mx[3] = { -3e38f, -3e38f, -3e38f };
+          for (size_t i = 0; i < scene.tri_verts.size(); ++i) { const int a = (int)(i % 3); mn[a] = std::min(mn[a], scene.tri_verts[i]); mx[a] = std::max(mx[a], scene.tri_verts[i]); }
+          for (int a = 0; a < 3; ++a) diag2 += ((double)mx[a] - mn[a]) * ((double)mx[a] - mn[a]); }
+        uint64_t budget = 4000000000ull;
+        if (const char* e = getenv("MI355RT_REFLECT_MASK_WORK")) budget = std::strtoull(e, nullptr, 10);
+        ReflMask rm;
+        if (std::isfinite(diag2) && build_reflect_mask(scene.tri_verts.data(), ntri, 2e-4 * std::sqrt(diag2) + 1e-7, kReflBins, budget, rm)) {
+            if (!upload(d_refl_mask, rm.words.data(), rm.words.size() * sizeof(uint32_t))) return bail();
+            refl_bins = rm.bins; refl_stride = rm.stride;
+            reflect_mask_info_[2] = (double)rm.clear_bits / ((double)ntri * 6.0 * rm.bins * rm.bins);
+            reflect_mask_info_[3] = (double)(rm.words.size() * sizeof(uint32_t));
+        }
+        reflect_mask_info_[0] = (double)refl_bins; reflect_mask_info_[1] = rm.build_ms;
+        if (getenv("MI355RT_DEBUG_CULL")) fprintf(stderr, "[mi355rt] reflection masks: %u bins per face edge, %.1f ms, %llu work units, %.3f of the bits clear\n", refl_bins, rm.build_ms, (unsigned long long)rm.work, reflect_mask_info_[2]);
+    }
     std::vector<DTexture> tex(std::max<size_t>(scene.textures.size(), 1));
     std::vector<float> texels;
     for (size_t i = 0; i < scene.textures.size(); ++i) {
@@ -237,6 +256,7 @@
     dscene_.lights = d_lights; dscene_.textures = d_tex; dscene_.texels = d_texels; dscene_.table = d_table;
     dscene_.root = bvh.root; dscene_.nlights = nlights_; dscene_.ntri = ntri;
     dscene_.light_maps = d_light_maps; dscene_.light_map_res = light_map_res;
+    dscene_.refl_mask = d_refl_mask; dscene_.refl_bins = refl_bins; dscene_.refl_stride = refl_stride;
     dscene_.oct_nodes = nullptr; dscene_.oct_leaf_tris = nullptr; dscene_.prim_tris = nullptr; dscene_.oct_info = nullptr; dscene_.tri_home = nullptr; dscene_.oct_single_leaf = 0u;
     std::memset(dscene_.oct_root, 0, sizeof dscene_.oct_root);
     mode_ = (cfg.flags & MI355RT_FLAG_OCTREE_SEMANTICS) ? kModeOctreeWalk : (cfg.flags & MI355RT_FLAG_TRUE_CLOSEST_HIT) ? kModeTrueClosest : kModeConfirm;
@@ -789,13 +809,15 @@
         const DCounters& s = shard[i];
         c.bounce += s.bounce; c.shadow += s.shadow; c.primary_hits += s.primary_hits;
         c.nodes_visited += s.nodes_visited; c.tris_tested += s.tris_tested; c.overflow |= s.overflow;
-        c.inner_execs += s.inner_execs; c.leaf_execs += s.leaf_execs; c.primary_culled += s.primary_culled; c.shadow_skipped += s.shadow_skipped;
-        c.t_sum_cycles += s.t_sum_cycles; c.t_sum_real += s.t_sum_real;
+        c.inner_execs += s.inner_execs; c.leaf_execs += s.leaf_execs; c.primary_culled += s.primary_culled; c.shadow_skipped += s.shadow_skipped; c.bounce_skipped += s.bounce_skipped;
+        c.t_sum_cycles += s.t_sum_cycles; c.t_sum_real += s.t_sum_real; c.refill_rays += s.refill_rays;
         for (int k = 0; k < 6; ++k) c.visits_below[k] += s.visits_below[k];
     }
     counts = mi355rt_ray_counts{};
-    counts.primary = primary; counts.bounce = c.bounce; counts.shadow = c.shadow + c.shadow_skipped; counts.primary_hits = c.primary_hits;
+    counts.primary = primary; counts.bounce = c.bounce + c.bounce_skipped; counts.shadow = c.shadow + c.shadow_skipped; counts.primary_hits = c.primary_hits;
     counts.shadow_skipped = c.shadow_skipped;
+    counts.bounce_skipped = c.bounce_skipped;
+    rays_read_ = c.refill_rays;
     counts.nodes_visited = c.nodes_visited; counts.tris_tested = c.tris_tested; counts.trace_launches = launches_;
     counts.inner_execs = c.inner_execs; counts.leaf_execs = c.leaf_execs; counts.primary_culled = c.primary_culled;
     if (getenv("MI355RT_DEBUG_UTIL") && c.nodes_visited)
diff --git a/raytracer-rs_amd/csrc/renderer.hpp b/raytracer-rs_amd/csrc/renderer.hpp
--- a/raytracer-rs_amd/csrc/renderer.hpp
+++ b/raytracer-rs_amd/csrc/renderer.hpp
@@ -93,6 +93,8 @@
     uint32_t oct_stats_[8] = { 0 };
     double build_ms_[2] = { 0.0, 0.0 };
     double light_map_ms_ = 0.0;
+    uint64_t rays_read_ = 0;
+    double reflect_mask_info_[4] = { 0.0, 0.0, 0.0, 0.0 };
     bool bvh_on_device_ = false;
     bool wide_ = false;
     uint32_t traversal_rows() const { return (wide_ ? bvh.stack_need4 : bvh.max_depth) + 1u; }
```

Result: faster. 20500, median of 6 (+10.6%).
